# psc0628/NeRF-PRV

Hardware: AMD Instinct MI355X
Metric: ray-samples/s (field evaluations composited; candidate views rendered + scored; scene baseline, field 256^3) (higher is better)
Workload: dtype f16

## Files before the change

### include/prv.h

```cpp
#ifndef PRV_H
#define PRV_H
#include <stddef.h>
#include <stdint.h>

#ifdef __cplusplus
extern "C" {
#endif

#define PRV_ABI_VERSION 5

#define PRV_OK 0
#define PRV_E_INVALID (-1)
#define PRV_E_HIP (-2)
#define PRV_E_IO (-3)
#define PRV_E_NODEVICE (-4)
#define PRV_E_STATE (-5)
#define PRV_E_INTERNAL (-6)

#define PRV_SCORE_ENSEMBLE_RGB 2
#define PRV_SCORE_ENSEMBLE_RGB_DENSITY 3
#define PRV_SCORE_PSNR_COVERAGE 5
#define PRV_SCORE_RAY_ENTROPY 7
#define PRV_SCORE_TERMINATION_JSD 9
#define PRV_TERMINATION_BINS_DEFAULT 16
// ... 241 lines not shown
typedef struct prv_coverage_opts {
  int32_t point_size;
  float depth_tol;
} prv_coverage_opts;
int prv_coverage_default_opts(prv_coverage_opts* opts);
int prv_coverage_create(prv_ctx* ctx, const float* xyz_dev, uint64_t n_points, const prv_camset* cs, const int* view_ids,
                        int n_views, int width, int height, const prv_coverage_opts* opts, float* depth_out_dev,
                        prv_coverage** out);
int prv_coverage_info(const prv_coverage* cov, uint64_t* n_points, int* n_views, uint64_t* n_coverable);
int prv_coverage_visible(const prv_coverage* cov, uint64_t* per_view_host);
int prv_coverage_bits(const prv_coverage* cov, int view, uint64_t* words_host);
int prv_coverage_curve(prv_coverage* cov, const int* order, int k, uint64_t* covered_host, uint32_t* first_seen_dev);
int prv_coverage_greedy(prv_coverage* cov, int k, int* chosen_out, uint64_t* covered_host);
void prv_coverage_destroy(prv_coverage* cov);

int prv_mesh_from_arrays(prv_ctx* ctx, const float* xyz_host, uint64_t n_vertices, const uint32_t* tri_host, uint64_t n_triangles,
                         prv_mesh** out);
int prv_mesh_depth(prv_ctx* ctx, const prv_mesh* m, const prv_camset* cs, const int* view_ids, int n_views, int width, int height,
                   float* depth_out_dev);
int prv_coverage_create_occluded(prv_ctx* ctx, const float* xyz_dev, uint64_t n_points, const prv_mesh* occluder, const prv_camset* cs,
                                 const int* view_ids, int n_views, int width, int height, const prv_coverage_opts* opts,
                                 float* depth_out_dev, prv_coverage** out);

int prv_mesh_set_colors(prv_mesh* m, const uint8_t* rgb_host, uint64_t n_vertices);
int prv_mesh_render(prv_ctx* ctx, const prv_mesh* m, const prv_camset* cs, const int* view_ids, int n_views, int width, int height,
                    int flip180, uint8_t* out_rgba8_dev, float* depth_out_dev, uint32_t* tri_out_dev);

typedef struct prv_comm prv_comm;
int prv_comm_create(prv_ctx* ctx, int rank, int world, const char* transport, const char* rendezvous, prv_comm** out);
void prv_comm_destroy(prv_comm* comm);
int prv_comm_rank(const prv_comm* comm);
int prv_comm_world(const prv_comm* comm);
const char* prv_comm_transport(const prv_comm* comm);
int prv_comm_library(const prv_comm* comm, char* path_out, int path_cap, int* version_out, char* how_out, int how_cap);
int prv_comm_all_gather(prv_comm* comm, const void* send_dev, size_t bytes_per_rank, void* recv_dev);
int prv_comm_barrier(prv_comm* comm);
int prv_shard_views(int n_views, int rank, int world, int interleaved, int* ids_out, int* n_mine);
int prv_score_views_sharded(prv_ctx* ctx, prv_comm* comm, int method, const int* model_slots, int n_models,
                            const prv_camset* cs, int n_views_total, int interleaved, const prv_render_opts* opts,
                            const float* gt_shard_dev, prv_score_record* records_host, prv_stats* stats);
int prv_model_exchange(prv_ctx* ctx, prv_comm* comm, int n_members, const prv_field_desc* desc);
int prv_model_exchange_slots(prv_ctx* ctx, prv_comm* comm, int n_members, const int* slots, const int* owners,
                             const prv_field_desc* desc);

typedef struct prv_train_opts {
  int32_t n_rays;
  int32_t n_samples;
  float lr, beta1, beta2, eps, l2_reg;
  float min_T;
  uint64_t seed;
  int32_t random_bg;
  int32_t occ_every;
  float occ_decay, occ_sigma_thresh;
  int32_t target_samples;
  int32_t patch_w, patch_h;
  int32_t step_mode;
  int32_t deterministic;
} prv_train_opts;
typedef struct prv_trainer prv_trainer;
int prv_train_default_opts(prv_train_opts* opts);
int prv_train_create(prv_ctx* ctx, int model_slot, const prv_camset* dataset, const uint8_t* images_rgba8_dev,
                     int width, int height, const prv_train_opts* opts, prv_trainer** out);
int prv_train_steps(prv_trainer* t, int n_steps, float* losses_host);
int prv_train_steps_multi(prv_trainer** trainers, int n_trainers, int n_steps, float* losses_host);
int prv_train_info(const prv_trainer* t, uint32_t* steps_done, uint64_t* samples_last_batch,
                   uint64_t* table_scalars);
int prv_train_active_rays(const prv_trainer* t);
void prv_train_destroy(prv_trainer* t);
int prv_train_gradients(prv_trainer* t, float* table_grad_host, float* mlp_grad_host, float* loss);
int prv_train_master(prv_trainer* t, float* table_host, float* mlp_host);
int prv_train_refresh_occupancy(prv_trainer* t);
int prv_train_debug_stamps(prv_trainer* t, unsigned long long* out64);

typedef struct prv_model_layout {
  uint64_t table_bytes_canonical;
  uint64_t table_bytes_physical;
  int32_t kernel_features;
  int32_t kernel_dense_levels;
  int32_t n_hashed_levels;
  int32_t kernel_slots;
  int32_t n_dense_levels;
} prv_model_layout;
int prv_debug_model_layout(prv_ctx* ctx, int model_slot, prv_model_layout* out);
int prv_debug_render_clock(prv_ctx* ctx, uint64_t* shader_cycles, uint64_t* ref_ticks, double* ref_hz);
int prv_debug_raygen(prv_ctx* ctx, const prv_camset* cs, int view, int width, int height,
                     int spp_index, float* o, float* d, float* t);
int prv_debug_mesh_stages(prv_ctx* ctx, float ms[4]);
int prv_debug_mesh_component_rounds(const prv_mesh* m, int* rounds);
int prv_debug_raster_stats(prv_ctx* ctx, uint64_t out[2]);
uint64_t prv_debug_live_bytes(void);
int prv_debug_encode(prv_ctx* ctx, int model_slot, const float* pos, int n, uint16_t* feat);
int prv_debug_field(prv_ctx* ctx, int model_slot, const float* pos, const float* dir, int n,
                    float* out36, int32_t* occupied);

#ifdef __cplusplus
}
#endif
#endif
```

### nerf_prv_amd/_lib.py

```python
import ctypes as C
import os

_HERE = os.path.dirname(os.path.abspath(__file__))
LIB_PATH = os.path.join(_HERE, "libprv_hip.so")

PRV_OK = 0
PRV_E_INVALID = -1
PRV_E_HIP = -2
PRV_E_IO = -3
PRV_E_NODEVICE = -4
PRV_E_STATE = -5
PRV_E_INTERNAL = -6

SCORE_ENSEMBLE_RGB = 2
SCORE_ENSEMBLE_RGB_DENSITY = 3
SCORE_PSNR_COVERAGE = 5
SCORE_RAY_ENTROPY = 7
SCORE_TERMINATION_JSD = 9
TERMINATION_BINS_DEFAULT = 16
STEP_FIXED_S = 0
STEP_NGP = 1
NGP_MAX_STEPS = 1024

NN_GRID = 0
# ... 139 lines not shown
    "prv_render_depth": (_i, [_vp, _i, _vp, _vp, _i, _P(RenderOpts), _vp, _vp, _P(Stats)]),
    "prv_render_entropy": (_i, [_vp, _i, _vp, _vp, _i, _P(RenderOpts), _vp, _vp, _P(Stats)]),
    "prv_render_termination": (_i, [_vp, _i, _vp, _vp, _i, _P(RenderOpts), _i, _vp, _vp, _P(Stats)]),
    "prv_termination_divergence": (_i, [_vp, _vp, _vp, _i, _i, _i, _i, _i, _vp, _vp, _vp]),
    "prv_render_footprint": (_i, [_vp, _i, _vp, _vp, _i, _P(RenderOpts), _vp, _vp, _vp, _P(Stats)]),
    "prv_render_surface": (_i, [_vp, _i, _vp, _vp, _i, _P(RenderOpts), C.c_float, _vp, _vp, _vp, _vp, _P(Stats)]),
    "prv_select_default_opts": (_i, [_P(SelectOpts)]),
    "prv_select_from_images": (_i, [_vp, _vp, _vp, _i, _i, _i, _vp, _vp, _vp, _P(SelectOpts), _vp, _vp, _vp, _vp]),
    "prv_select_views": (_i, [_vp, _i, _vp, _vp, _i, _P(RenderOpts), _P(SelectOpts), _vp, _vp, _P(Stats)]),
    "prv_select_views_surface": (_i, [_vp, _i, _vp, _vp, _i, _P(RenderOpts), C.c_float, _P(SelectOpts), _vp, _vp, _P(Stats)]),
    "prv_first_hit": (_i, [_vp, _i, _vp, _vp, _i, _i, _i, C.c_float, _vp]),
    "prv_precept": (_i, [_vp, _i, _vp, _i, _vp, _P(Rs2Intrinsics), C.c_float, _vp]),
    "prv_quantize_rgba8": (_i, [_vp, _vp, C.c_size_t, _vp, _vp]),
    "prv_mesh_default_opts": (_i, [_P(MeshOpts)]),
    "prv_density_grid": (_i, [_vp, _i, _P(MeshOpts), _vp]),
    "prv_marching_cubes": (_i, [_vp, _i, _P(MeshOpts), _P(_vp)]),
    "prv_marching_cubes_grid": (_i, [_vp, _vp, _P(MeshOpts), _P(_vp)]),
    "prv_mesh_counts": (_i, [_vp, _P(C.c_uint64), _P(C.c_uint64)]),
    "prv_mesh_get": (_i, [_vp, _vp, _vp, _vp, _vp]),
    "prv_mesh_save": (_i, [_vp, C.c_char_p, C.c_double, _vp]),
    "prv_mesh_write_file": (_i, [C.c_char_p, C.c_uint64, _vp, _vp, _vp, C.c_uint64, _vp, C.c_double, _vp]),
    "prv_mesh_destroy": (None, [_vp]),
    "prv_mesh_filter_default_opts": (_i, [_P(MeshFilterOpts)]),
    "prv_mesh_components": (_i, [_vp, _P(C.c_uint64)]),
    "prv_mesh_component_info": (_i, [_vp, C.c_uint64, _vp]),
    "prv_mesh_labels": (_i, [_vp, _vp, _vp]),
    "prv_mesh_filter": (_i, [_vp, _P(MeshFilterOpts), _P(_vp)]),
    "prv_mesh_sample": (_i, [_vp, C.c_uint64, C.c_uint64, _vp, _vp]),
    "prv_nn_default_opts": (_i, [_P(NNOpts)]),
    "prv_nn_index_create": (_i, [_vp, _vp, C.c_uint64, _P(NNOpts), _P(_vp)]),
    "prv_nn_query": (_i, [_vp, _vp, C.c_uint64, _vp, _vp]),
    "prv_nn_index_info": (_i, [_vp, _P(C.c_uint64), _P(C.c_int32), _P(C.c_int32)]),
    "prv_debug_nn_tests": (_i, [_vp, _P(C.c_uint64)]),
    "prv_nn_index_destroy": (None, [_vp]),
    "prv_geometry_metrics": (_i, [_vp, _vp, C.c_uint64, _vp, C.c_uint64, C.c_float, _P(GeomMetrics)]),
    "prv_geometry_metrics_indexed": (_i, [_vp, _vp, C.c_uint64, _vp, _vp, C.c_uint64, C.c_float, _P(GeomMetrics)]),
    "prv_coverage_default_opts": (_i, [_P(CoverageOpts)]),
    "prv_coverage_create": (_i, [_vp, _vp, C.c_uint64, _vp, _vp, _i, _i, _i, _P(CoverageOpts), _vp, _P(_vp)]),
    "prv_coverage_info": (_i, [_vp, _P(C.c_uint64), _P(_i), _P(C.c_uint64)]),
    "prv_coverage_visible": (_i, [_vp, _vp]),
    "prv_coverage_bits": (_i, [_vp, _i, _vp]),
    "prv_coverage_curve": (_i, [_vp, _vp, _i, _vp, _vp]),
    "prv_coverage_greedy": (_i, [_vp, _i, _vp, _vp]),
    "prv_coverage_destroy": (None, [_vp]),
    "prv_mesh_from_arrays": (_i, [_vp, _vp, C.c_uint64, _vp, C.c_uint64, _P(_vp)]),
    "prv_mesh_depth": (_i, [_vp, _vp, _vp, _vp, _i, _i, _i, _vp]),
    "prv_mesh_set_colors": (_i, [_vp, _vp, C.c_uint64]),
    "prv_mesh_render": (_i, [_vp, _vp, _vp, _vp, _i, _i, _i, _i, _vp, _vp, _vp]),
    "prv_coverage_create_occluded": (_i, [_vp, _vp, C.c_uint64, _vp, _vp, _vp, _i, _i, _i, _P(CoverageOpts), _vp, _P(_vp)]),
    "prv_debug_raster_stats": (_i, [_vp, _vp]),
    "prv_debug_live_bytes": (C.c_uint64, []),
    "prv_score_ensemble_images": (_i, [_vp, _i, _vp, _i, _i, C.c_size_t, _vp]),
    "prv_score_psnr_images": (_i, [_vp, _vp, _vp, _i, C.c_size_t, _vp, _vp]),
    "prv_evaluate_images": (_i, [_vp, _vp, _vp, _i, _i, _i, _vp, _vp, _vp]),
    "prv_evaluate": (_i, [_vp, _i, _vp, _vp, _i, _P(RenderOpts), _vp, _P(C.c_double), _P(C.c_double)]),
    "prv_score_views": (_i, [_vp, _i, _vp, _i, _vp, _vp, _i, _P(RenderOpts), _vp, _vp, _vp, _P(Stats)]),
    "prv_rank": (_i, [_vp, _vp, _i, _vp]),
    "prv_argmax": (_i, [_vp, _vp, _i]),
    "prv_splat_points": (_i, [_vp, _vp, _vp, C.c_size_t, C.c_double, _vp, _vp, _vp, _i, _i, _i, _i, _i, _vp]),
    "prv_train_default_opts": (_i, [_P(TrainOpts)]),
    "prv_train_create": (_i, [_vp, _i, _vp, _vp, _i, _i, _P(TrainOpts), _P(_vp)]),
    "prv_train_steps": (_i, [_vp, _i, _vp]),
    "prv_train_steps_multi": (_i, [_vp, _i, _i, _vp]),
    "prv_train_debug_stamps": (_i, [_vp, _vp]),
    "prv_train_info": (_i, [_vp, _P(C.c_uint32), _P(C.c_uint64), _P(C.c_uint64)]),
    "prv_train_active_rays": (_i, [_vp]),
    "prv_train_destroy": (None, [_vp]),
    "prv_train_gradients": (_i, [_vp, _vp, _vp, _P(C.c_float)]),
    "prv_train_master": (_i, [_vp, _vp, _vp]),
    "prv_train_refresh_occupancy": (_i, [_vp]),
    "prv_comm_create": (_i, [_vp, _i, _i, C.c_char_p, C.c_char_p, C.POINTER(_vp)]),
    "prv_comm_destroy": (None, [_vp]),
    "prv_comm_rank": (_i, [_vp]),
    "prv_comm_world": (_i, [_vp]),
    "prv_comm_transport": (C.c_char_p, [_vp]),
    "prv_comm_library": (_i, [_vp, C.c_char_p, _i, _P(_i), C.c_char_p, _i]),
    "prv_comm_all_gather": (_i, [_vp, _vp, C.c_size_t, _vp]),
    "prv_comm_barrier": (_i, [_vp]),
    "prv_shard_views": (_i, [_i, _i, _i, _i, _vp, C.POINTER(_i)]),
    "prv_score_views_sharded": (_i, [_vp, _vp, _i, _vp, _i, _vp, _i, _i, C.POINTER(RenderOpts), _vp, _vp, C.POINTER(Stats)]),
    "prv_model_exchange": (_i, [_vp, _vp, _i, C.POINTER(FieldDesc)]),
    "prv_model_exchange_slots": (_i, [_vp, _vp, _i, _P(_i), _P(_i), C.POINTER(FieldDesc)]),
    "prv_debug_model_layout": (_i, [_vp, _i, C.POINTER(ModelLayout)]),
    "prv_debug_render_clock": (_i, [_vp, C.POINTER(C.c_uint64), C.POINTER(C.c_uint64), C.POINTER(C.c_double)]),
    "prv_debug_raygen": (_i, [_vp, _vp, _i, _i, _i, _i, _vp, _vp, _vp]),
    "prv_debug_mesh_stages": (_i, [_vp, _P(C.c_float)]),
    "prv_debug_mesh_component_rounds": (_i, [_vp, _P(C.c_int)]),
    "prv_debug_encode": (_i, [_vp, _i, _vp, _i, _vp]),
    "prv_debug_field": (_i, [_vp, _i, _vp, _vp, _i, _vp, _vp]),
}

_lib = None


def load():
    global _lib
    if _lib is not None:
        return _lib
    if not os.path.exists(LIB_PATH):
        raise ImportError(
            f"{LIB_PATH} is missing: build it with `python -c 'import __graft_entry__ as g; g.build()'` "
            "(hipcc --offload-arch=gfx950). There is no CPU fallback for the render path."
        )
    lib = C.CDLL(LIB_PATH)
    for name, (res, args) in SIGNATURES.items():
        try:
            fn = getattr(lib, name)
        except AttributeError as e:
            raise ImportError(f"{LIB_PATH} does not export {name}") from e
        fn.restype = res
        fn.argtypes = args
    _lib = lib
    return lib


def device_code_digest(path=None):
    import hashlib
    import struct

    path = path or LIB_PATH
    with open(path, "rb") as fh:
        data = fh.read()
    if data[:4] != b"\x7fELF" or data[4] != 2:
        raise ValueError(f"{path} is not a 64-bit ELF file")
    shoff, = struct.unpack_from("<Q", data, 0x28)
    shentsize, shnum, shstrndx = struct.unpack_from("<HHH", data, 0x3A)
    sections = [struct.unpack_from("<IIQQQQIIQQ", data, shoff + i * shentsize) for i in range(shnum)]
    stroff = sections[shstrndx][4]
    for name_off, _type, _flags, _addr, off, size, *_ in sections:
        end = data.index(b"\0", stroff + name_off)
        if data[stroff + name_off:end] == b".hip_fatbin":
            return hashlib.sha256(data[off:off + size]).hexdigest()[:16]
    raise ValueError(f"{path} has no .hip_fatbin section")
```

### nerf_prv_amd/api.py

```python
import ctypes as C
import enum
import json
import math

import numpy as np

from . import _lib as L

RECORD_DTYPE = np.dtype([("score", "<f8"), ("psnr", "<f4"), ("coverage", "<f4")])

FIELD_256 = dict(n_levels=8, n_features=4, log2_hashmap=19, base_res=16, finest_res=256, occ_res=128,
                 density_bias=3.0, table_amp=4.0)
FIELD_512 = dict(n_levels=16, n_features=2, log2_hashmap=21, base_res=16, finest_res=512, occ_res=128,
                 density_bias=3.0, table_amp=4.0)
FIELD_HBM = dict(n_levels=16, n_features=2, log2_hashmap=24, base_res=16, finest_res=2048, occ_res=128,
                 density_bias=3.0, table_amp=4.0)


class RenderMode(enum.IntEnum):

    Shade = 0
    Depth = 1


Shade, Depth = RenderMode.Shade, RenderMode.Depth


class PrvError(RuntimeError):
    def __init__(self, code, msg):
        super().__init__(f"prv error {code}: {msg}")
        self.code = code


def field_desc(**kw):
    d = dict(FIELD_256)
    d.update(kw)
    return L.FieldDesc(**d)


def render_opts(width, height, samples_per_ray=128, spp=1, min_transmittance=1e-4, background=(0.0, 0.0, 0.0, 0.0),
                step_mode=L.STEP_FIXED_S):
    o = L.RenderOpts()
    o.width, o.height, o.samples_per_ray, o.spp = int(width), int(height), int(samples_per_ray), int(spp)
    o.step_mode = int(step_mode)
    o.min_transmittance = float(min_transmittance)
    for k in range(4):
        o.background[k] = float(background[k])
    return o


def engine_render_opts(width, height, samples_per_ray, spp, min_transmittance, background=(0.0, 0.0, 0.0, 0.0)):
    n = int(samples_per_ray)
    return render_opts(width, height, n, spp, min_transmittance, background, step_mode=L.STEP_NGP if n == 0 else L.STEP_FIXED_S)


def select_opts(k=None, grid_res=None, alpha_min=None):
    o = L.SelectOpts()
    if L.load().prv_select_default_opts(C.byref(o)) != 0:
        raise PrvError(L.PRV_E_INVALID, "prv_select_default_opts failed")
    if k is not None:
        o.k = int(k)
    if grid_res is not None:
        o.grid_res = int(grid_res)
    if alpha_min is not None:
        o.alpha_min = float(alpha_min)
    return o


def model_sizes(desc):
    lib = L.load()
    t, m, o = C.c_uint64(), C.c_uint64(), C.c_uint64()
    rc = lib.prv_model_sizes(C.byref(desc), C.byref(t), C.byref(m), C.byref(o))
    if rc != 0:
        raise PrvError(rc, "invalid field descriptor")
    return t.value, m.value, o.value


def _ptr(a):
    if a is None:
        return None
    if isinstance(a, np.ndarray):
        return a.ctypes.data_as(C.c_void_p)
    return C.c_void_p(a.data_ptr())


class _Handle:
    _destroy = None

    def __init__(self, ctx, handle):
        self.ctx, self.handle = ctx, handle

    def _chk(self, rc):
        if rc != 0:
            lib = self.ctx.lib
            msg = (lib.prv_last_error(self.ctx.handle) if self.ctx.handle else None) or b""
            if not (self.handle and msg) or rc == L.PRV_E_STATE:
                msg = lib.prv_last_error(None) or msg
            raise PrvError(rc, msg.decode())

# ... 1101 lines not shown
```

### nerf_prv_amd/csrc/prv_api.cpp

```cpp
#include <hip/hip_runtime.h>

#include <algorithm>
#include <atomic>
#include <chrono>
#include <cmath>
#include <cstdarg>
#include <cstdio>
#include <cstdlib>
#include <cstring>
#include <memory>
#include <new>
#include <stdexcept>
#include <string>
#include <vector>

#include "prv_buffer.hpp"
#include "prv_json.hpp"
#include "prv_kernels.hpp"
#include "prv_mesh.hpp"
#include "prv_geom.hpp"
#include "prv_select.hpp"
#include "prv_coverage.hpp"
#include "prv_raster.hpp"
#include "prv_levels.hpp"
#include "prv_ingp.hpp"
#include "prv_train.hpp"
#include "prv_train_switches.hpp"

using namespace prv;


namespace {

thread_local std::string g_create_error;
std::atomic<int> g_live_contexts{0};
std::atomic<unsigned long long> g_devices_used{0};
std::atomic<bool> g_rccl_loaded{false};

struct Model {
  bool loaded = false;
  bool dirty = false;
  uint64_t generation = 0;
  prv_field_desc desc{};
  FieldDev dev{};
  uint64_t table_halfs = 0, occ_words = 0;
  uint64_t phys_bytes = 0;
  float occ_lo[3] = {0, 0, 0}, occ_hi[3] = {1, 1, 1};
  Buffer table, phys, occ, occ_coarse, frags, frags64, mlp;
};

}

struct prv_camset {
  std::vector<CamDev> cams;
  CamDev* dev = nullptr;
  int device = 0;
  int width = 0, height = 0;
  bool dataset = false;
};

using prv_handle = prv::Handle<struct prv_ctx>;

struct prv_ctx {
  int device = 0;
  int n_cu = 256;
  hipStream_t own_stream = nullptr;
  hipStream_t stream = nullptr;
  std::vector<hipStream_t> idle_queues;
  hipStream_t capture_stream = nullptr;
  BufferPool parked;
  std::string err;
  Model models[PRV_MAX_SLOTS];
  Buffer queue, queue_ext, stage, counters, view_ids, img_f32, partial, records, dbg[6];
  Buffer stage_depth;
  Buffer stage_foot;
  Buffer stage_hit;
  Buffer stage_bins;
  Buffer term_planes;
  Buffer sel_planes, sel_voxel, sel_q, sel_bits, sel_sums;
  Buffer counters_multi, occ_multi;
  int march_multi = -1;
  Buffer img_u8[PRV_MAX_MODELS];
  bool profiling = false;
  std::vector<hipEvent_t> ev_render, ev_march;
  std::vector<hipEvent_t> ev_free;
  std::vector<float> last_render_ms;
  void* pin = nullptr;
  size_t pin_cap = 0;
  hipEvent_t pin_ev = nullptr;
  int blocks_per_cu = -1;
  int cell_cache = -1;
  std::vector<prv_handle*> handles;
  uint64_t raster_stats[2] = {0, 0};
  float mesh_ms[4] = {0, 0, 0, 0};
  int queue_segments = 8;
  int spatial_regions = 1;
  int pool_on = -1;
  int merge_max = -1;
  size_t stage_budget = (size_t)4 << 30;
  size_t queue_budget = (size_t)8 << 30;
  double coverage_weight = PRV_COVERAGE_WEIGHT_DEFAULT;
};

namespace {

int fail(prv_ctx* c, int code, const char* fmt, ...) {
  char buf[512];
  va_list ap;
  va_start(ap, fmt);
  vsnprintf(buf, sizeof(buf), fmt, ap);
  va_end(ap);
  if (c) c->err = buf;
  else g_create_error = buf;
  return code;
}

int caught(prv_ctx* c) noexcept {
  try {
    throw;
  } catch (const std::bad_alloc&) {
    try {
      return fail(c, PRV_E_INTERNAL, "out of host memory");
    } catch (...) {
      return PRV_E_INTERNAL;
    }
  } catch (const std::exception& e) {
    try {
      return fail(c, PRV_E_INTERNAL, "internal error: %s", e.what());
    } catch (...) {
      return PRV_E_INTERNAL;
    }
  } catch (...) {
    return PRV_E_INTERNAL;
  }
}

#define HIPCHK(c, expr)                                                                           \
  do {                                                                                            \
    hipError_t e__ = (expr);                                                                      \
    if (e__ != hipSuccess) return fail((c), PRV_E_HIP, "%s failed: %s", #expr, hipGetErrorString(e__)); \
  } while (0)

int ensure(prv_ctx* c, Buffer& b, size_t bytes) {
  const char* call = "";
  const hipError_t e = prv::ensure(b, bytes, c->stream, c->parked, &call);
  if (e != hipSuccess) return fail(c, PRV_E_HIP, "%s failed: %s", call, hipGetErrorString(e));
  return PRV_OK;
}

int handle_alive(const prv_handle* h, const char* name, const char* the_name) {
  if (!h) return fail(nullptr, PRV_E_INVALID, "%s is NULL", name);
  if (!h->ctx) return fail(nullptr, PRV_E_STATE, "%s's context has been destroyed", the_name);
  return PRV_OK;
}

static_assert(kMaxFieldLevels == kMaxLevels, "level tables of the host and the kernels must agree");

const int kIn[5] = {32, 64, 32, 64, 64};
const int kOut[5] = {64, 16, 64, 64, 16};
const int kOff[5] = {0, 2048, 3072, 5120, 9216};

inline int hidden_k(int s, int h, int j) { return 32 * (s >> 1) + 16 * (s & 1) + 8 * (j >> 2) + 4 * h + (j & 3); }

void prepack_fragments(const uint16_t* mlp, int n_features, std::vector<uint16_t>& frags, bool v64 = false) {
  frags.assign((size_t)kNumFrags * kFragHalfs, 0);
  int f = 0;
  auto emit = [&](int layer, int mt, int s, int (*kmap)(int, int, int)) {
    uint16_t* dst = frags.data() + (size_t)f * kFragHalfs;
    for (int lane = 0; lane < 64; lane++) {
      const int r = lane & 31, h = lane >> 5;
      int out = 32 * mt + r;
      if (v64 && (layer == 1 || layer == 4) && out >= 20 && out < 20 + (layer == 1 ? 1 : 3)) out -= 20;
      for (int j = 0; j < 8; j++) {
        const int k = kmap(s, h, j);
        dst[lane * 8 + j] = out < kOut[layer] ? mlp[kOff[layer] + k * kOut[layer] + out] : (uint16_t)0;
      }
    }
    f++;
  };
  auto k_feat4 = [](int s, int h, int j) { return 4 * (2 * (s * 2 + j / 4) + h) + j % 4; };
  auto k_feat2 = [](int s, int h, int j) { return 2 * (2 * (s * 4 + j / 2) + h) + j % 2; };
  auto k_rgb_in = [](int s, int h, int j) { return s == 0 ? hidden_k(0, h, j) : 16 + 8 * h + j; };
  auto k_canon = [](int s, int h, int j) { return 16 * s + 8 * h + j; };
  for (int mt = 0; mt < 2; mt++)
    for (int s = 0; s < 2; s++)
      emit(0, mt, s, v64 ? (int (*)(int, int, int))k_canon : n_features == 4 ? (int (*)(int, int, int))k_feat4 : (int (*)(int, int, int))k_feat2);
  for (int s = 0; s < 4; s++) emit(1, 0, s, hidden_k);
  for (int mt = 0; mt < 2; mt++)
    for (int s = 0; s < 2; s++) emit(2, mt, s, k_rgb_in);
  for (int mt = 0; mt < 2; mt++)
    for (int s = 0; s < 4; s++) emit(3, mt, s, hidden_k);
  for (int s = 0; s < 4; s++) emit(4, 0, s, hidden_k);
}

uint16_t f2h(float f) {
  _Float16 h = (_Float16)f;
  uint16_t u;
  memcpy(&u, &h, 2);
  return u;
}
uint64_t mix64(uint64_t z) {
  z = (z ^ (z >> 30)) * 0xBF58476D1CE4E5B9ull;
  z = (z ^ (z >> 27)) * 0x94D049BB133111EBull;
  return z ^ (z >> 31);
}
float rng_sym(uint64_t seed, uint64_t stream, uint64_t i, float amp) {
  const uint64_t hsh = mix64(seed + (stream + 1) * 0xD1B54A32D192ED03ull + i * 0x9E3779B97F4A7C15ull);
  const uint32_t u = (uint32_t)(hsh >> 40);
  const float v = (float)u * (1.0f / 8388608.0f) - 1.0f;
  return v * amp;
}
const float kSynthSpheres[4][4] = {
    {0.50f, 0.50f, 0.50f, 0.35f}, {0.80f, 0.50f, 0.62f, 0.13f}, {0.36f, 0.80f, 0.45f, 0.11f}, {0.40f, 0.24f, 0.78f, 0.10f}};

int install_model(prv_ctx* c, int slot, const prv_field_desc& d, const uint16_t* mlp, const uint32_t* occ_host,
                  const uint16_t* table_host ) {
  Model& m = c->models[slot];
  HostLevel lv[kMaxLevels];
  uint64_t total = 0;
  if (compute_levels(d, lv, &total) != 0) return fail(c, PRV_E_INVALID, "invalid field descriptor");
  m.loaded = false;
  m.desc = d;
  m.table_halfs = total * (uint64_t)d.n_features;
  const uint64_t R = (uint64_t)d.occ_res;
  m.occ_words = (R * R * R + 31) / 32;
  int rc;
  if ((rc = ensure(c, m.table, m.table_halfs * 2)) != PRV_OK) return rc;
  if ((rc = ensure(c, m.occ, m.occ_words * 4)) != PRV_OK) return rc;
  if ((rc = ensure(c, m.frags, (size_t)kNumFrags * kFragHalfs * 2)) != PRV_OK) return rc;
  if ((rc = ensure(c, m.frags64, (size_t)kNumFrags * kFragHalfs * 2)) != PRV_OK) return rc;
  if ((rc = ensure(c, m.mlp, PRV_MLP_HALFS * 2)) != PRV_OK) return rc;
  if (table_host) HIPCHK(c, hipMemcpyAsync(m.table.p, table_host, m.table_halfs * 2, hipMemcpyHostToDevice, c->stream));
  HIPCHK(c, hipMemcpyAsync(m.occ.p, occ_host, m.occ_words * 4, hipMemcpyHostToDevice, c->stream));
  {
    const int R = d.occ_res;
    int lo[3] = {R, R, R}, hi[3] = {-1, -1, -1};
    const bool words = R % 32 == 0;
    for (int z = 0; words && z < R; z++)
      for (int y = 0; y < R; y++)
        for (int w = 0; w < R / 32; w++) {
          const uint32_t v = occ_host[((size_t)R * ((size_t)y + (size_t)R * (size_t)z)) / 32 + (size_t)w];
          if (!v) continue;
          lo[0] = std::min(lo[0], 32 * w + __builtin_ctz(v));
          hi[0] = std::max(hi[0], 32 * w + 31 - __builtin_clz(v));
          lo[1] = std::min(lo[1], y);
          hi[1] = std::max(hi[1], y);
          lo[2] = std::min(lo[2], z);
          hi[2] = std::max(hi[2], z);
        }
    for (int z = 0; !words && z < R; z++)
      for (int y = 0; y < R; y++)
        for (int x = 0; x < R; x++) {
          const size_t b = (size_t)x + (size_t)R * ((size_t)y + (size_t)R * (size_t)z);
          if (!((occ_host[b >> 5] >> (b & 31)) & 1u)) continue;
          const int cxyz[3] = {x, y, z};
          for (int a = 0; a < 3; a++) {
            lo[a] = std::min(lo[a], cxyz[a]);
            hi[a] = std::max(hi[a], cxyz[a]);
          }
        }
    for (int a = 0; a < 3; a++) {
      m.occ_lo[a] = hi[a] < 0 ? 2.0f : (float)(lo[a] - 1) / (float)R;
      m.occ_hi[a] = hi[a] < 0 ? -1.0f : (float)(hi[a] + 2) / (float)R;
    }
  }
  std::vector<uint32_t> coarse;
  if (d.occ_res % 4 == 0 && d.occ_res >= 8) {
    const int R = d.occ_res, Rc = R / 4;
    std::vector<uint8_t> blk((size_t)Rc * Rc * Rc, 0);
    const bool words = R % 32 == 0;
    for (int z = 0; words && z < R; z++)
      for (int y = 0; y < R; y++)
        for (int w = 0; w < R / 32; w++) {
          const uint32_t v = occ_host[((size_t)R * ((size_t)y + (size_t)R * (size_t)z)) / 32 + (size_t)w];
          if (!v) continue;
          uint8_t* row = &blk[(size_t)(8 * w) + (size_t)Rc * ((size_t)(y / 4) + (size_t)Rc * (size_t)(z / 4))];
          for (int k = 0; k < 8; k++)
            if ((v >> (4 * k)) & 0xfu) row[k] = 1;
        }
    for (int z = 0; !words && z < R; z++)
      for (int y = 0; y < R; y++)
        for (int x = 0; x < R; x += 32) {
          const size_t bit0 = (size_t)x + (size_t)R * ((size_t)y + (size_t)R * (size_t)z);
          for (int k = 0; k < 32 && x + k < R; k++) {
            const size_t b = bit0 + k;
            if ((occ_host[b >> 5] >> (b & 31)) & 1u) blk[(size_t)((x + k) / 4) + (size_t)Rc * ((size_t)(y / 4) + (size_t)Rc * (size_t)(z / 4))] = 1;
          }
        }
    coarse.assign(((size_t)Rc * Rc * Rc + 31) / 32, 0u);
    for (int z = 0; z < Rc; z++)
      for (int y = 0; y < Rc; y++)
        for (int x = 0; x < Rc; x++) {
          bool any = false;
          for (int dz = -1; dz <= 1 && !any; dz++)
            for (int dy = -1; dy <= 1 && !any; dy++)
              for (int dx = -1; dx <= 1 && !any; dx++) {
// ... 22 lines not shown
  auto ceil_log2 = [](uint32_t v) { uint32_t s = 0; while ((1u << s) < v) s++; return s; };
  for (int l = 0; l < d.n_levels; l++) {
    order[l] = l;
    if (lv[l].hashed) {
      sx[l] = 0;
      psize[l] = lv[l].size;
    } else {
      sx[l] = ceil_log2(lv[l].res + 1);
      psize[l] = 1u << ceil_log2((lv[l].res + 1u) << (2 * sx[l]));
    }
  }
  std::stable_sort(order, order + d.n_levels, [&](int a, int b) { return psize[a] > psize[b]; });
  uint64_t ptotal = 0;
  for (int k = 0; k < d.n_levels; k++) {
    poff[order[k]] = (uint32_t)ptotal;
    ptotal += psize[order[k]];
  }
  if (ptotal * ebytes >= (1ull << 32)) return fail(c, PRV_E_INVALID, "field too large for 32-bit gather offsets");
  if ((rc = ensure(c, m.phys, ptotal * ebytes)) != PRV_OK) return rc;
  m.phys_bytes = ptotal * ebytes;
  HIPCHK(c, hipMemsetAsync(m.phys.p, 0, ptotal * ebytes, c->stream));
  for (int l = 0; l < d.n_levels; l++) {
    RepackLevel R{lv[l].offset, poff[l], lv[l].size, lv[l].res, sx[l], lv[l].hashed};
    HIPCHK(c, launch_repack_level((const uint16_t*)m.table.p, (uint16_t*)m.phys.p, R, d.n_features, c->stream));
  }
  HIPCHK(c, hipStreamSynchronize(c->stream));
  FieldDev& f = m.dev;
  memset(&f, 0, sizeof(f));
  f.table = (const uint16_t*)m.phys.p;
  f.occ = (const uint32_t*)m.occ.p;
  f.occ_coarse = (d.occ_res % 4 == 0 && d.occ_res >= 8) ? (const uint32_t*)m.occ_coarse.p : nullptr;
  f.frags = (const half8*)m.frags.p;
  f.frags64 = (const half8*)m.frags64.p;
  f.n_levels = d.n_levels;
  f.n_features = d.n_features;
  f.occ_res = d.occ_res;
  f.density_bias = d.density_bias;
  for (int a = 0; a < 3; a++) {
    f.occ_lo[a] = m.occ_lo[a];
    f.occ_hi[a] = m.occ_hi[a];
  }
  f.n_dense_levels = 0;
  while (f.n_dense_levels < d.n_levels && !lv[f.n_dense_levels].hashed) f.n_dense_levels++;
  if (getenv("PRV_NO_PAIR")) f.n_dense_levels = 0;
  f.hash_my_b = (2654435761u * ebytes) & 0xffffffu;
  f.hash_mz_b = (805459861u * ebytes) & 0xffffffu;
  f.hash_m_b = (uint32_t)(((1ull << d.log2_hashmap) - 1ull) * ebytes);
  f.hash_shared = 1;
  f.wide_offsets = 0;
  for (int l = 0; l < d.n_levels; l++)
    if (lv[l].hashed && (lv[l].res > lv[l].size || l < f.n_dense_levels)) f.hash_shared = 0;
  if (getenv("PRV_NO_PAIR")) f.hash_shared = 0;
  for (int l = 0; l < d.n_levels; l++) {
    LevelDev& L = f.levels[l];
    L.scale = lv[l].scale;
    L.res_m1 = lv[l].res - 1;
    if (lv[l].res > 4096) return fail(c, PRV_E_INVALID, "level %d has %u vertices per axis (limit 4096)", l, lv[l].res);
    if (lv[l].hashed) {
      if ((uint64_t)(lv[l].size - 1u) * ebytes >= (1ull << 32)) return fail(c, PRV_E_INVALID, "hashed level of 4 GiB or more");
      L.m_b = (lv[l].size - 1u) * ebytes;
      const bool wide = L.m_b >= (1u << 24);
      L.my_b = wide ? 2654435761u * ebytes : (2654435761u * ebytes) & 0xffffffu;
      L.mz_b = wide ? 805459861u * ebytes : (805459861u * ebytes) & 0xffffffu;
      if (wide) {
        f.wide_offsets = 1;
        f.hash_shared = 0;
      }
    } else {
      L.my_b = ebytes << sx[l];
      L.mz_b = ebytes << (2 * sx[l]);
      L.m_b = 0xffffffffu;
      if (L.mz_b >= (1u << 24) || lv[l].res > 4096) return fail(c, PRV_E_INVALID, "dense level too large");
    }
    L.off_b = poff[l] * ebytes;
    L.myz_b = L.my_b + L.mz_b;
    if (lv[l].hashed) {
      if ((L.off_b & 4095u) != 0u || L.res_m1 > 4095u) f.hash_shared = 0;
      L.pack = (L.off_b & ~4095u) | (L.res_m1 & 4095u);
    } else {
      if ((L.off_b & 31u) != 0u || sx[l] > 31u) f.hash_shared = 0;
      L.pack = (L.off_b & ~31u) | (sx[l] & 31u);
    }
  }
  m.loaded = true;
  m.dirty = false;
  return PRV_OK;
}

int republish_model(prv_ctx* c, int slot) {
  Model& m = c->models[slot];
  HIPCHK(c, hipSetDevice(c->device));
  std::vector<uint16_t> mlp(PRV_MLP_HALFS);
  std::vector<uint32_t> occ(m.occ_words);
  HIPCHK(c, hipMemcpyAsync(mlp.data(), m.mlp.p, PRV_MLP_HALFS * 2, hipMemcpyDeviceToHost, c->stream));
  HIPCHK(c, hipMemcpyAsync(occ.data(), m.occ.p, m.occ_words * 4, hipMemcpyDeviceToHost, c->stream));
  HIPCHK(c, hipStreamSynchronize(c->stream));
  const prv_field_desc d = m.desc;
  return install_model(c, slot, d, mlp.data(), occ.data(), nullptr);
}

int model_present(prv_ctx* c, int slot) {
  if (slot < 0 || slot >= PRV_MAX_SLOTS) return fail(c, PRV_E_INVALID, "model slot %d out of range", slot);
  if (!c->models[slot].loaded) return fail(c, PRV_E_STATE, "model slot %d is empty", slot);
  return PRV_OK;
}

int republish_model(prv_ctx* c, int slot);

int check_model(prv_ctx* c, int slot) {
  int rc = model_present(c, slot);
  if (rc != PRV_OK) return rc;
  if (c->models[slot].dirty) return republish_model(c, slot);
  return PRV_OK;
}

int check_opts(prv_ctx* c, const prv_render_opts* o) {
  if (!o) return fail(c, PRV_E_INVALID, "render options are NULL");
  if (o->width < 1 || o->height < 1 || o->width > 16384 || o->height > 16384)
    return fail(c, PRV_E_INVALID, "bad image size %dx%d", o->width, o->height);
  if (o->step_mode != PRV_STEP_FIXED_S && o->step_mode != PRV_STEP_NGP)
    return fail(c, PRV_E_INVALID, "step_mode must be PRV_STEP_FIXED_S (0) or PRV_STEP_NGP (1), got %d", o->step_mode);
  if (o->step_mode == PRV_STEP_FIXED_S && (o->samples_per_ray < 1 || o->samples_per_ray > kMaxSamples))
    return fail(c, PRV_E_INVALID, "samples_per_ray must be in [1,%d], got %d", kMaxSamples, o->samples_per_ray);
  if (o->spp < 1 || o->spp > 1024) return fail(c, PRV_E_INVALID, "spp must be in [1,1024], got %d", o->spp);
  return PRV_OK;
}

int check_surface_level(prv_ctx* c, const prv_render_opts* o, float level) {
  if (!(level > 0.0f && level < 1.0f)) return fail(c, PRV_E_INVALID, "level must be in (0, 1), got %g", (double)level);
  if (1.0f - level < o->min_transmittance)
    return fail(c, PRV_E_INVALID, "level %g: 1 - level = %g is below min_transmittance %g, rays would be cut before they can cross", (double)level,
                (double)(1.0f - level), (double)o->min_transmittance);
  return PRV_OK;
}

int check_device_ptr(prv_ctx* c, const void* p, const char* what) {
  if (!p) return PRV_OK;
  hipPointerAttribute_t a;
  if (hipPointerGetAttributes(&a, p) != hipSuccess) {
    (void)hipGetLastError();
    return fail(c, PRV_E_INVALID, "%s is not a device pointer", what);
  }
  if (a.type != hipMemoryTypeDevice && a.type != hipMemoryTypeManaged && a.type != hipMemoryTypeUnified)
    return fail(c, PRV_E_INVALID, "%s is not a device pointer", what);
  return PRV_OK;
}

hipError_t take_event(prv_ctx* c, hipEvent_t* e) {
  if (!c->ev_free.empty()) {
    *e = c->ev_free.back();
    c->ev_free.pop_back();
    return hipSuccess;
  }
  return hipEventCreate(e);
}

CamDev cam_at(const prv_camset* cs, int i, int w, int h) {
  const CamDev& c = cs->cams[i];
  CamDev r = c;
  const float s = (float)w / (float)cs->width;
  if (cs->dataset) {
    const float sy = (float)h / (float)cs->height;
    r.fx = c.fx * s;
    r.fy = c.fy * sy;
    r.cx = c.cx * s;
    r.cy = c.cy * sy;
// ... 264 lines not shown
    if (!term) planes[n_planes++] = {t.entropy, &c->stage_depth, &RenderPlanesParams::out_entropy};
    planes[n_planes++] = {t.alpha, &c->stage, &RenderPlanesParams::out_alpha};
  }
  const size_t n_bins = term ? (size_t)t.n_bins : 0;
  if (depth) planes[n_planes++] = {t.depth, colour ? &c->stage_depth : &c->stage_foot, &RenderPlanesParams::out_depth};
  if (surface) planes[n_planes++] = {t.hit, &c->stage_hit, &RenderPlanesParams::out_hit};
  const size_t stage_px = (colour ? 16 : 0) + 4 * ((size_t)n_planes + n_bins);
  if (spp > 1) batch = std::min<size_t>(batch, std::max<size_t>(1, c->stage_budget / (npix * stage_px * (size_t)spp)));
  if (batch * npix * (size_t)spp >= (1ull << 32)) batch = ((1ull << 32) - 1) / (npix * (size_t)spp);
  if (batch == 0) return fail(c, PRV_E_INVALID, "image x spp too large");
  const MarchLayout L(c, W, H, spp);
  const size_t seg_cap_max = L.seg_cap(batch);
  if (seg_cap_max * (size_t)L.n_seg >= (1ull << 32)) return fail(c, PRV_E_INVALID, "image x spp too large");
  if ((rc = ensure(c, c->queue, seg_cap_max * (size_t)L.n_seg * kRecordBytes)) != PRV_OK) return rc;
  if (ngp && (rc = ensure(c, c->queue_ext, seg_cap_max * (size_t)L.n_seg * kExtBytes)) != PRV_OK) return rc;
  if (spp > 1 && colour && (rc = ensure(c, c->stage, batch * npix * (size_t)spp * 16)) != PRV_OK) return rc;
  for (int i = 0; i < n_planes && spp > 1; i++)
    if ((rc = ensure(c, *planes[i].stage, batch * npix * (size_t)spp * 4)) != PRV_OK) return rc;
  if (term && spp > 1 && (rc = ensure(c, c->stage_bins, n_bins * batch * npix * (size_t)spp * 4)) != PRV_OK) return rc;

  const int n_blocks = render_blocks(c, m, npix);
  for (size_t b0 = 0; b0 < (size_t)n_views; b0 += batch) {
    const int nb = (int)std::min(batch, (size_t)n_views - b0);
    float* dst_f32 = t.rgba ? t.rgba + b0 * npix * 4 : nullptr;
    uint32_t* dst_u8 = t.rgba8 ? (uint32_t*)t.rgba8 + b0 * npix : nullptr;
    float *dst[4], *target[4];
    for (int i = 0; i < n_planes; i++) {
      dst[i] = planes[i].out + b0 * npix;
      target[i] = spp > 1 ? (float*)planes[i].stage->p : dst[i];
      HIPCHK(c, hipMemsetAsync(target[i], 0, (size_t)nb * npix * (size_t)spp * 4, c->stream));
    }
    const size_t bins_stride = spp > 1 ? (size_t)nb * npix * (size_t)spp : t.bins_stride;
    float* const bins_target = !term ? nullptr : spp > 1 ? (float*)c->stage_bins.p : t.bins + b0 * npix;
    const size_t plane_px = (size_t)nb * npix * (size_t)spp;
    if (n_bins && bins_stride == plane_px) HIPCHK(c, hipMemsetAsync(bins_target, 0, n_bins * plane_px * 4, c->stream));
    else
      for (size_t k = 0; k < n_bins; k++) HIPCHK(c, hipMemsetAsync(bins_target + k * bins_stride, 0, plane_px * 4, c->stream));
    HIPCHK(c, hipMemsetAsync(c->counters.p, 0, b0 == 0 && t.zero_stats ? kCountersBytes : kStatOffset, c->stream));
    MarchParams mp;
    march_common(mp, c, L, o, up, b0, (size_t)nb, stat);
    mp.field = m.dev;
    mp.S = o->samples_per_ray;
    mp.step_mode = o->step_mode;
    mp.queue = c->queue.p;
    mp.queue_ext = (uint4*)c->queue_ext.p;
    mp.queue_count = q_count;
    mp.out_f32 = !colour ? nullptr : spp > 1 ? (float*)c->stage.p : dst_f32;
    mp.out_u8 = spp > 1 ? nullptr : dst_u8;
    if (private_output) {
      const uint64_t tw = 1ull << mp.tile_w_log2, th = 1ull << mp.tile_h_log2;
      uint64_t live_max = 0;
      for (int i = 0; i < nb; i++) {
        const CamDev& cv = up.cams[b0 + i];
        uint64_t w = mp.tiles_x, h = mp.tiles_y;
        if (cv.cull[2] > 0) {
          const uint64_t x0 = (uint64_t)cv.cull[0] / tw, y0 = (uint64_t)cv.cull[1] / th;
          const uint64_t x1 = std::min<uint64_t>(mp.tiles_x, ((uint64_t)cv.cull[2] + tw - 1) / tw);
          const uint64_t y1 = std::min<uint64_t>(mp.tiles_y, ((uint64_t)std::max(cv.cull[3], 0) + th - 1) / th);
          w = x1 > x0 ? x1 - x0 : 0;
          h = y1 > y0 ? y1 - y0 : 0;
        }
        live_max = std::max(live_max, w * h);
      }
      mp.live_grid = 1;
      mp.live_tiles_max = (uint32_t)live_max;
    }
    if ((rc = timed(c, c->ev_march, [&] { HIPCHK(c, launch_march(mp, nb, spp, c->stream)); return PRV_OK; })) != PRV_OK) return rc;
    RenderPlanesParams pp;
    memset(&pp, 0, sizeof(pp));
    pp.r = render_params(c, m, o, L, mp.seg_cap, {mp.queue, mp.queue_ext, mp.queue_count, mp.out_f32, mp.out_u8}, q_head, stat, t.mode);
    for (int i = 0; i < n_planes; i++) pp.*planes[i].slot = target[i];
    pp.cams = mp.cams;
    pp.view_ids = mp.view_ids;
    pp.npix = (uint32_t)npix;
    pp.nb = (uint32_t)nb;
    pp.T_cross = 1.0f - t.level;
    if (term) {
      pp.out_bins = bins_target;
      pp.plane_stride = bins_stride;
      pp.n_bins = (uint32_t)n_bins;
      pp.bin_mul = (uint32_t)(n_bins * 65536u / (size_t)(ngp ? kNgpMaxSteps : o->samples_per_ray));
    }
    if ((rc = timed(c, c->ev_render, [&] {
           HIPCHK(c, n_planes ? launch_render_planes(pp, t.mode, n_blocks, c->stream) : launch_render(pp.r, n_blocks, c->stream));
           return PRV_OK;
         })) != PRV_OK)
      return rc;
    if (spp > 1 && colour) HIPCHK(c, launch_spp_reduce((const float*)c->stage.p, (size_t)nb * npix, spp, o->background, dst_f32, dst_u8, c->stream));
    for (int i = 0; i < n_planes && spp > 1; i++) HIPCHK(c, launch_spp_reduce_depth(target[i], (size_t)nb * npix, spp, dst[i], c->stream));
    for (size_t k = 0; k < n_bins && spp > 1; k++)
      HIPCHK(c, launch_spp_reduce_depth(bins_target + k * bins_stride, (size_t)nb * npix, spp, t.bins + k * t.bins_stride + b0 * npix, c->stream));
  }
  return PRV_OK;
}

int render_ensemble_ngp(prv_ctx* c, const int* slots, int E, const prv_camset* cs, const int* view_ids, int n_views,
                        const prv_render_opts* o, float* scratch_f32, uint8_t* const* out_u8, bool* done) {
  *done = false;
  if (o->step_mode != PRV_STEP_NGP || !march_multi_supported(E) || n_views == 0) return PRV_OK;
  if (c->march_multi == 0) return PRV_OK;
  if (c->march_multi < 0 && E < 3) return PRV_OK;
  const Model& m0 = c->models[slots[0]];
  for (int e = 1; e < E; e++) {
    const Model& m = c->models[slots[e]];
    if (m.desc.occ_res != m0.desc.occ_res || (m.dev.occ_coarse == nullptr) != (m0.dev.occ_coarse == nullptr)) return PRV_OK;
    for (int f = 0; f < e; f++)
      if (slots[f] == slots[e]) return PRV_OK;
  }
  const int W = o->width, H = o->height, spp = o->spp;
  const size_t npix = (size_t)W * H;
  const size_t slot_bytes = kRecordBytes + kExtBytes;
  if ((size_t)n_views * npix * (size_t)spp >= (1ull << 32)) return PRV_OK;
  if ((size_t)n_views * npix * (size_t)spp * slot_bytes > c->queue_budget) return PRV_OK;
  if (spp > 1 && (size_t)n_views * npix * (size_t)spp * 16 > c->stage_budget) return PRV_OK;
  const MarchLayout L(c, W, H, spp);
  const size_t seg_cap = L.seg_cap((size_t)n_views);
  if (seg_cap * (size_t)L.n_seg >= (1ull << 32)) return PRV_OK;
  int rc;
  if ((rc = ensure(c, c->counters, kCountersBytes)) != PRV_OK) return rc;
  if ((rc = ensure(c, c->counters_multi, (size_t)E * kStatOffset)) != PRV_OK) return rc;
  unsigned long long* stat = (unsigned long long*)((char*)c->counters.p + kStatOffset);
  const size_t R = (size_t)m0.desc.occ_res, n_fine = R * R * R, Rc = R / 4, n_coarse = Rc * Rc * Rc;
  if ((rc = ensure(c, c->occ_multi, n_fine + n_coarse + 64)) != PRV_OK) return rc;
  const size_t q_stride = seg_cap * (size_t)L.n_seg * kRecordBytes, x_stride = seg_cap * (size_t)L.n_seg * kExtBytes,
               s_stride = spp > 1 ? (size_t)n_views * npix * (size_t)spp * 16 : 0;
  {
    const size_t grow = (q_stride * (size_t)E > c->queue.bytes ? q_stride * (size_t)E - c->queue.bytes : 0) +
                        (x_stride * (size_t)E > c->queue_ext.bytes ? x_stride * (size_t)E - c->queue_ext.bytes : 0) +
                        (s_stride * (size_t)E > c->stage.bytes ? s_stride * (size_t)E - c->stage.bytes : 0);
    size_t free_b = 0, total_b = 0;
    if (grow && (hipMemGetInfo(&free_b, &total_b) != hipSuccess || grow + ((size_t)2 << 30) > free_b + c->parked.bytes)) return PRV_OK;
  }

  const OccBox box = union_box(c, slots, E);
  Upload up;
  if ((rc = upload_views(c, cs, view_ids, n_views, W, H, box, up)) != PRV_OK) return rc;

  const bool have_coarse = m0.dev.occ_coarse != nullptr;
  {
    OccInterleaveParams ip{};
    ip.n_members = E;
    for (int e = 0; e < E; e++) ip.bits[e] = c->models[slots[e]].dev.occ;
    ip.n_cells = (uint32_t)n_fine;
    ip.out = (uint8_t*)c->occ_multi.p;
    HIPCHK(c, launch_occ_interleave(ip, c->stream));
    if (have_coarse) {
      for (int e = 0; e < E; e++) ip.bits[e] = c->models[slots[e]].dev.occ_coarse;
      ip.n_cells = (uint32_t)n_coarse;
      ip.out = (uint8_t*)c->occ_multi.p + n_fine;
      HIPCHK(c, launch_occ_interleave(ip, c->stream));
    }
  }

  if ((rc = ensure(c, c->queue, q_stride * (size_t)E)) != PRV_OK) return rc;
  if ((rc = ensure(c, c->queue_ext, x_stride * (size_t)E)) != PRV_OK) return rc;
  if (spp > 1 && (rc = ensure(c, c->stage, s_stride * (size_t)E)) != PRV_OK) return rc;
  HIPCHK(c, hipMemsetAsync(c->counters.p, 0, kCountersBytes, c->stream));
  HIPCHK(c, hipMemsetAsync(c->counters_multi.p, 0, (size_t)E * kStatOffset, c->stream));

  MarchMultiParams mp;
  march_common(mp, c, L, o, up, 0, (size_t)n_views, stat);
  mp.occ_bytes = (const uint8_t*)c->occ_multi.p;
  mp.occ_coarse_bytes = have_coarse ? (const uint8_t*)c->occ_multi.p + n_fine : nullptr;
  mp.occ_res = (int)R;
  for (int a = 0; a < 3; a++) {
    mp.occ_lo[a] = box.occ_lo[a];
    mp.occ_hi[a] = box.occ_hi[a];
  }
  mp.n_members = E;
  for (int e = 0; e < E; e++) {
    MarchMember& mm = mp.mem[e];
    mm.queue = (char*)c->queue.p + q_stride * (size_t)e;
    mm.queue_ext = (uint4*)((char*)c->queue_ext.p + x_stride * (size_t)e);
    mm.queue_count = (uint32_t*)((char*)c->counters_multi.p + (size_t)e * kStatOffset) + kMaxSegments * 16;
    mm.out_f32 = spp > 1 ? (float*)((char*)c->stage.p + s_stride * (size_t)e) : scratch_f32;
    mm.out_u8 = spp > 1 ? nullptr : (uint32_t*)out_u8[e];
  }
  if ((rc = timed(c, c->ev_march, [&] { HIPCHK(c, launch_march_multi(mp, n_views, spp, c->stream)); return PRV_OK; })) != PRV_OK) return rc;

  for (int e = 0; e < E; e++) {
    const Model& m = c->models[slots[e]];
    const int n_blocks = render_blocks(c, m, npix);
    uint32_t* q_head = (uint32_t*)((char*)c->counters_multi.p + (size_t)e * kStatOffset);
    const RenderParams rp = render_params(c, m, o, L, mp.seg_cap, mp.mem[e], q_head, stat, kRenderColour);
    if ((rc = timed(c, c->ev_render, [&] { HIPCHK(c, launch_render(rp, n_blocks, c->stream)); return PRV_OK; })) != PRV_OK) return rc;
    if (spp > 1)
      HIPCHK(c, launch_spp_reduce((const float*)mp.mem[e].out_f32, (size_t)n_views * npix, spp, o->background, scratch_f32, (uint32_t*)out_u8[e], c->stream));
  }
  *done = true;
  return PRV_OK;
}

int fetch_stats(prv_ctx* c, const prv_render_opts* o, int n_views, int n_models, prv_stats* st) {
  if (!st) return PRV_OK;
  unsigned long long ev[72] = {0};
  HIPCHK(c, hipMemcpyAsync(ev, (char*)c->counters.p + kStatOffset, sizeof(ev), hipMemcpyDeviceToHost, c->stream));
  HIPCHK(c, hipStreamSynchronize(c->stream));
  st->wave_rounds = ev[1];
  st->rays = (uint64_t)n_views * n_models * o->width * o->height * o->spp;
  st->samples_nominal = st->rays * (uint64_t)(o->step_mode == PRV_STEP_NGP ? kNgpMaxSteps : o->samples_per_ray);
  st->samples_evaluated = ev[0];
  st->samples_live = 0;
  for (int s = 0; s < 8; s++) st->samples_live += ev[8 * (1 + s)];
  return PRV_OK;
}

struct NamedPtr {
  const void* p;
  const char* name;
};
int render_entry(prv_ctx* c, int slot, const prv_camset* cs, const int* view_ids, int n_views, const prv_render_opts* o, prv_stats* st,
                 RenderTargets t, std::initializer_list<NamedPtr> outs, bool missing, const char* bad,
                 float* RenderTargets::*scratch = nullptr, size_t scratch_px = 0) {
  if (!c) return PRV_E_INVALID;
  int rc;
  if ((rc = check_model(c, slot)) != PRV_OK || (rc = check_opts(c, o)) != PRV_OK) return rc;
  if (!cs || n_views < 0 || (missing && n_views > 0)) return fail(c, PRV_E_INVALID, "%s", bad);
  HIPCHK(c, hipSetDevice(c->device));
  for (const NamedPtr& out : outs)
    if ((rc = check_device_ptr(c, out.p, out.name)) != PRV_OK) return rc;
  if (scratch && !(t.*scratch) && n_views > 0) {
    if ((rc = ensure(c, c->img_f32, (size_t)n_views * o->width * o->height * scratch_px)) != PRV_OK) return rc;
    t.*scratch = (float*)c->img_f32.p;
  }
  if ((rc = render_views(c, slot, cs, view_ids, n_views, o, t)) != PRV_OK) return rc;
  return fetch_stats(c, o, n_views, 1, st);
}

int score_blocks(size_t npix) { return (int)std::min<size_t>(64, std::max<size_t>(1, (npix + 4095) / 4096)); }

}


extern "C" {

int prv_abi_version(void) { return PRV_ABI_VERSION; }

int prv_device_count(void) {
  int n = 0;
  if (hipGetDeviceCount(&n) != hipSuccess) return 0;
  return n;
}

const char* prv_last_error(const prv_ctx* ctx) { return ctx ? ctx->err.c_str() : g_create_error.c_str(); }

int prv_create(prv_ctx** out, int device_id) try {
  if (!out) return fail(nullptr, PRV_E_INVALID, "out is NULL");
  *out = nullptr;
  int n = 0;
  hipError_t e = hipGetDeviceCount(&n);
  if (e != hipSuccess || n <= 0)
    return fail(nullptr, PRV_E_NODEVICE, "no HIP device visible (%s): this library has no CPU path",
                e == hipSuccess ? "count = 0" : hipGetErrorString(e));
  if (device_id < 0 || device_id >= n) return fail(nullptr, PRV_E_INVALID, "device %d out of range [0,%d)", device_id, n);
  hipDeviceProp_t prop;
  if ((e = hipSetDevice(device_id)) != hipSuccess || (e = hipGetDeviceProperties(&prop, device_id)) != hipSuccess)
    return fail(nullptr, PRV_E_HIP, "device %d: %s", device_id, hipGetErrorString(e));
  if (!strstr(prop.gcnArchName, "gfx950"))
    return fail(nullptr, PRV_E_NODEVICE, "device %d is %s; this library is built for gfx950 only", device_id, prop.gcnArchName);
  prv_ctx* c = new prv_ctx();
  c->device = device_id;
  c->n_cu = prop.multiProcessorCount > 0 ? prop.multiProcessorCount : 256;
  if ((e = hipStreamCreateWithFlags(&c->own_stream, hipStreamNonBlocking)) != hipSuccess) {
    delete c;
    return fail(nullptr, PRV_E_HIP, "stream create: %s", hipGetErrorString(e));
  }
  c->stream = c->own_stream;
  if (const char* s = getenv("PRV_BLOCKS_PER_CU")) c->blocks_per_cu = std::max(1, atoi(s));
// ... 927 lines not shown
    if (n_views && (rc = score_ensemble_dev(c, method, imgs, n_models, n_views, npix, rec)) != PRV_OK) return rc;
  } else {
    const bool priv = o->spp == 1;
    RenderTargets t;
    t.rgba = (float*)c->img_f32.p;
    t.private_output = priv;
    if ((rc = render_views(c, model_slots[0], cs, view_ids, n_views, o, t)) != PRV_OK) return rc;
    if (n_views && (rc = score_psnr_dev(c, (const float*)c->img_f32.p, gt, n_views, npix, o->background, c->coverage_weight, rec,
                                        priv ? (const CamDev*)c->view_ids.p : nullptr, o->width)) != PRV_OK)
      return rc;
  }
  if (rec_dev && n_views)
    HIPCHK(c, hipMemcpyAsync(rec_dev, rec, (size_t)n_views * sizeof(prv_score_record), hipMemcpyDeviceToDevice, c->stream));
  if (rec_host && n_views) {
    HIPCHK(c, hipMemcpyAsync(rec_host, rec, (size_t)n_views * sizeof(prv_score_record), hipMemcpyDeviceToHost, c->stream));
    HIPCHK(c, hipStreamSynchronize(c->stream));
  }
  return fetch_stats(c, o, n_views, n_models, st);
} catch (...) { return caught(c); }

int prv_argmax(const prv_score_record* r, const int* ids, int n) {
  if (!r || !ids) return -1;
  double best = -1e100;
  int best_id = -1;
  for (int i = 0; i < n; i++)
    if (r[i].score > best) {
      best = r[i].score;
      best_id = ids[i];
    }
  return best_id;
}

int prv_rank(const prv_score_record* r, const int* ids, int n, int* order) try {
  if (n < 0 || (n > 0 && (!r || !ids || !order))) return PRV_E_INVALID;
  std::vector<int> idx(n);
  for (int i = 0; i < n; i++) idx[i] = i;
  std::stable_sort(idx.begin(), idx.end(), [&](int a, int b) {
    const bool na = std::isnan(r[a].score), nb = std::isnan(r[b].score);
    if (na != nb) return nb;
    if (!na && r[a].score != r[b].score) return r[a].score > r[b].score;
    return ids[a] < ids[b];
  });
  for (int i = 0; i < n; i++) order[i] = ids[idx[i]];
  return PRV_OK;
} catch (...) { return caught(nullptr); }


int prv_debug_render_clock(prv_ctx* c, uint64_t* shader_cycles, uint64_t* ref_ticks, double* ref_hz) try {
  if (!c) return PRV_E_INVALID;
  HIPCHK(c, hipSetDevice(c->device));
  if (!shader_cycles || !ref_ticks || !ref_hz) return fail(c, PRV_E_INVALID, "NULL output");
  if (!c->counters.p) return fail(c, PRV_E_STATE, "nothing rendered yet");
  unsigned long long v[2] = {0, 0};
  HIPCHK(c, hipMemcpyAsync(v, (char*)c->counters.p + kStatOffset + 16, 16, hipMemcpyDeviceToHost, c->stream));
  HIPCHK(c, hipStreamSynchronize(c->stream));
  int khz = 0;
  HIPCHK(c, hipDeviceGetAttribute(&khz, hipDeviceAttributeWallClockRate, c->device));
  *shader_cycles = v[0];
  *ref_ticks = v[1];
  *ref_hz = (double)khz * 1e3;
  return PRV_OK;
} catch (...) { return caught(c); }

int prv_debug_model_layout(prv_ctx* c, int slot, prv_model_layout* out) try {
  if (!c) return PRV_E_INVALID;
  int rc = check_model(c, slot);
  if (rc != PRV_OK) return rc;
  if (!out) return fail(c, PRV_E_INVALID, "out is NULL");
  const Model& m = c->models[slot];
  HostLevel lv[kMaxLevels];
  uint64_t total = 0;
  compute_levels(m.desc, lv, &total);
  out->table_bytes_canonical = m.table_halfs * 2;
  out->table_bytes_physical = m.phys_bytes;
  out->kernel_features = m.dev.n_features;
  out->kernel_dense_levels = render_instance_dense_levels(m.dev);
  out->kernel_slots = 64;
  out->n_dense_levels = m.dev.n_dense_levels;
  out->n_hashed_levels = 0;
  for (int l = 0; l < m.desc.n_levels; l++) out->n_hashed_levels += lv[l].hashed ? 1 : 0;
  return PRV_OK;
} catch (...) { return caught(c); }

int prv_debug_raygen(prv_ctx* c, const prv_camset* cs, int view, int W, int H, int spp_k, float* o, float* d, float* t) try {
  if (!c) return PRV_E_INVALID;
  if (!cs || view < 0 || view >= (int)cs->cams.size() || W < 1 || H < 1 || !o || !d || !t)
    return fail(c, PRV_E_INVALID, "bad argument");
  HIPCHK(c, hipSetDevice(c->device));
  const size_t n = (size_t)W * H;
  int rc;
  if ((rc = ensure(c, c->dbg[0], n * 12)) != PRV_OK || (rc = ensure(c, c->dbg[1], n * 12)) != PRV_OK ||
      (rc = ensure(c, c->dbg[2], n * 8)) != PRV_OK)
    return rc;
  HIPCHK(c, launch_debug_raygen(cam_at(cs, view, W, H), W, H, spp_k, (float*)c->dbg[0].p,
                                (float*)c->dbg[1].p, (float*)c->dbg[2].p, c->stream));
  HIPCHK(c, hipMemcpyAsync(o, c->dbg[0].p, n * 12, hipMemcpyDeviceToHost, c->stream));
  HIPCHK(c, hipMemcpyAsync(d, c->dbg[1].p, n * 12, hipMemcpyDeviceToHost, c->stream));
  HIPCHK(c, hipMemcpyAsync(t, c->dbg[2].p, n * 8, hipMemcpyDeviceToHost, c->stream));
  HIPCHK(c, hipStreamSynchronize(c->stream));
  return PRV_OK;
} catch (...) { return caught(c); }

static int debug_field_common(prv_ctx* c, int slot, const float* pos, const float* dir, int n, uint16_t* feat,
                              float* out36, int32_t* occ) {
  int rc;
  if ((rc = check_model(c, slot)) != PRV_OK) return rc;
  if (n < 0 || (n > 0 && !pos)) return fail(c, PRV_E_INVALID, "bad argument");
  if (n == 0) return PRV_OK;
  HIPCHK(c, hipSetDevice(c->device));
  const size_t N = (size_t)n;
  if ((rc = ensure(c, c->dbg[0], N * 12)) != PRV_OK || (rc = ensure(c, c->dbg[1], N * 12)) != PRV_OK ||
      (rc = ensure(c, c->dbg[3], N * 64)) != PRV_OK || (rc = ensure(c, c->dbg[4], N * 144)) != PRV_OK ||
      (rc = ensure(c, c->dbg[5], N * 4)) != PRV_OK)
    return rc;
  HIPCHK(c, hipMemcpyAsync(c->dbg[0].p, pos, N * 12, hipMemcpyHostToDevice, c->stream));
  if (dir) HIPCHK(c, hipMemcpyAsync(c->dbg[1].p, dir, N * 12, hipMemcpyHostToDevice, c->stream));
  HIPCHK(c, launch_debug_field(c->models[slot].dev, (const float*)c->dbg[0].p, dir ? (const float*)c->dbg[1].p : nullptr,
                               n, (uint16_t*)c->dbg[3].p, (float*)c->dbg[4].p, (int32_t*)c->dbg[5].p, c->stream));
  if (feat) HIPCHK(c, hipMemcpyAsync(feat, c->dbg[3].p, N * 64, hipMemcpyDeviceToHost, c->stream));
  if (out36) HIPCHK(c, hipMemcpyAsync(out36, c->dbg[4].p, N * 144, hipMemcpyDeviceToHost, c->stream));
  if (occ) HIPCHK(c, hipMemcpyAsync(occ, c->dbg[5].p, N * 4, hipMemcpyDeviceToHost, c->stream));
  HIPCHK(c, hipStreamSynchronize(c->stream));
  return PRV_OK;
}

int prv_debug_encode(prv_ctx* c, int slot, const float* pos, int n, uint16_t* feat) try {
  if (!c) return PRV_E_INVALID;
  if (!feat && n > 0) return fail(c, PRV_E_INVALID, "feat is NULL");
  return debug_field_common(c, slot, pos, nullptr, n, feat, nullptr, nullptr);
} catch (...) { return caught(c); }

int prv_debug_field(prv_ctx* c, int slot, const float* pos, const float* dir, int n, float* out36, int32_t* occ) try {
  if (!c) return PRV_E_INVALID;
  if (n > 0 && (!dir || !out36)) return fail(c, PRV_E_INVALID, "NULL argument");
  return debug_field_common(c, slot, pos, dir, n, nullptr, out36, occ);
} catch (...) { return caught(c); }

}

#include "prv_train_api.inc"
#include "prv_comm_api.inc"
#include "prv_mesh_api.inc"
#include "prv_geom_api.inc"
#include "prv_select_api.inc"
#include "prv_raster_api.inc"
#include "prv_raster_color_api.inc"
#include "prv_coverage_api.inc"
```

### nerf_prv_amd/csrc/prv_device.hpp

```cpp
#pragma once
#include <utility>
#include <hip/hip_runtime.h>
#include <stdint.h>

namespace prv {

constexpr int kMaxLevels = 16;
constexpr int kNumFrags = 24;
constexpr int kFragHalfs = 64 * 8;
constexpr int kTile = 16;
constexpr int kChunkRays = kTile * kTile;
constexpr float kNgpDt = 1.7320508075688772f / 1024.0f;

typedef _Float16 half8 __attribute__((ext_vector_type(8)));
typedef _Float16 half4 __attribute__((ext_vector_type(4)));
typedef _Float16 half2v __attribute__((ext_vector_type(2)));
typedef float f32x16 __attribute__((ext_vector_type(16)));

struct LevelDev {
  float scale;
  uint32_t res_m1;
  uint32_t my_b, mz_b;
  uint32_t m_b;
  uint32_t off_b;
  uint32_t myz_b;
  uint32_t pack;
};

struct FieldDev {
  const uint16_t* table;
  const uint32_t* occ;
  const uint32_t* occ_coarse;
  const half8* frags;
  const half8* frags64;
  LevelDev levels[kMaxLevels];
  int n_levels, n_features, occ_res;
  int n_dense_levels;
  uint32_t hash_my_b, hash_mz_b, hash_m_b;
  int hash_shared;
  int wide_offsets;
  float density_bias;
  float occ_lo[3], occ_hi[3];
};

struct CamDev {
  float c2w[12];
  float fx, fy, cx, cy;
  float lens[4];
  int cull[4];
};


__device__ __forceinline__ float clamp01(float x) { return fminf(fmaxf(x, 0.0f), 1.0f); }

__device__ __forceinline__ void spp_offset(int k, float& ox, float& oy) {
  float fk = (float)k;
  float a = fmaf(fk, 0.7548776662466927f, 0.5f);
  float b = fmaf(fk, 0.5698402909980532f, 0.5f);
  ox = a - floorf(a);
  oy = b - floorf(b);
}

__device__ __forceinline__ void lens_eval(const float L[4], float x, float y, float& fx, float& fy, float J[4]) {
  const float k1 = L[0], k2 = L[1], p1 = L[2], p2 = L[3];
  const float r2 = fmaf(x, x, y * y);
  const float kr = fmaf(k2, r2, k1);
  const float radial = fmaf(kr, r2, 1.0f);
  const float dk = 2.0f * fmaf(2.0f * k2, r2, k1);
  const float xy = x * y;
  fx = fmaf(x, radial, fmaf(2.0f * p1, xy, p2 * fmaf(2.0f * x, x, r2)));
  fy = fmaf(y, radial, fmaf(p1, fmaf(2.0f * y, y, r2), (2.0f * p2) * xy));
  const float a = 2.0f * fmaf(p1, x, p2 * y);
  J[0] = fmaf(x * x, dk, fmaf(2.0f * p1, y, fmaf(6.0f * p2, x, radial)));
  J[1] = fmaf(xy, dk, a);
  J[2] = J[1];
  J[3] = fmaf(y * y, dk, fmaf(6.0f * p1, y, fmaf(2.0f * p2, x, radial)));
}

constexpr int kLensIters = 8;
__device__ __forceinline__ void lens_undistort(const float L[4], float& px, float& py) {
  const float xd = px, yd = py;
  float x = xd, y = yd;
  for (int it = 0; it < kLensIters; it++) {
    float fx, fy, J[4];
    lens_eval(L, x, y, fx, fy, J);
    const float ex = fx - xd, ey = fy - yd;
    const float det = fmaf(J[0], J[3], -(J[1] * J[2]));
    const float sx = fmaf(J[3], ex, -(J[1] * ey)) / det;
    const float sy = fmaf(J[0], ey, -(J[2] * ex)) / det;
    x -= sx;
    y -= sy;
  }
  px = x;
  py = y;
}

__device__ __forceinline__ bool has_lens(const CamDev& cam) {
  return cam.lens[0] != 0.0f || cam.lens[1] != 0.0f || cam.lens[2] != 0.0f || cam.lens[3] != 0.0f;
}

__device__ __forceinline__ void raygen(const CamDev& cam, int px, int py, float ox, float oy,
                                       float o[3], float d[3]) {
  float dx = (((float)px + ox) - cam.cx) / cam.fx;
  float dy = (((float)py + oy) - cam.cy) / cam.fy;
  if (has_lens(cam)) lens_undistort(cam.lens, dx, dy);
  float v[3];
#pragma unroll
  for (int r = 0; r < 3; r++) {
    const float* m = cam.c2w + r * 4;
    v[r] = fmaf(m[0], dx, fmaf(m[1], dy, m[2]));
    o[r] = m[3];
  }
  float n2 = fmaf(v[0], v[0], fmaf(v[1], v[1], v[2] * v[2]));
  float inv = 1.0f / sqrtf(n2);
#pragma unroll
  for (int r = 0; r < 3; r++) d[r] = v[r] * inv;
}

__device__ __forceinline__ void dataset_to_engine_point(float scale, const float off[3], const float* p, float e[3]) {
  const float q[3] = {fmaf(p[0], scale, off[0]), fmaf(p[1], scale, off[1]), fmaf(p[2], scale, off[2])};
  e[0] = q[1];
  e[1] = q[2];
  e[2] = q[0];
}

// ... 84 lines not shown
  point[0] = depth * x;
  point[1] = depth * y;
  point[2] = depth;
}

__device__ __forceinline__ _Float16 to_half(float x) {
  asm("" : "+v"(x));
  return (_Float16)x;
}

__device__ __forceinline__ void sh4(float x, float y, float z, float o[16]) {
  float xy = x * y, xz = x * z, yz = y * z, x2 = x * x, y2 = y * y, z2 = z * z;
  o[0] = 0.28209479177387814f;
  o[1] = -0.48860251190291987f * y;
  o[2] = 0.48860251190291987f * z;
  o[3] = -0.48860251190291987f * x;
  o[4] = 1.0925484305920792f * xy;
  o[5] = -1.0925484305920792f * yz;
  o[6] = 0.94617469575755997f * z2 - 0.31539156525251999f;
  o[7] = -1.0925484305920792f * xz;
  o[8] = 0.54627421529603959f * x2 - 0.54627421529603959f * y2;
  o[9] = (0.59004358992664352f * y) * (-3.0f * x2 + y2);
  o[10] = (2.8906114426405538f * xy) * z;
  o[11] = (0.45704579946446572f * y) * (1.0f - 5.0f * z2);
  o[12] = (0.3731763325901154f * z) * (5.0f * z2 - 3.0f);
  o[13] = (0.45704579946446572f * x) * (1.0f - 5.0f * z2);
  o[14] = (1.4453057213202769f * z) * (x2 - y2);
  o[15] = (0.59004358992664352f * x) * (-x2 + 3.0f * y2);
}

template <int F> struct EntryWord;
template <> struct EntryWord<4> { typedef uint2 type; };
template <> struct EntryWord<2> { typedef uint32_t type; };
template <int F> struct Entry;
template <> struct Entry<4> {
  uint32_t w[2];
  __device__ __forceinline__ static Entry load(const char* p) {
    const uint2 v = *reinterpret_cast<const uint2*>(p);
    Entry e;
    e.w[0] = v.x;
    e.w[1] = v.y;
    return e;
  }
};
template <> struct Entry<2> {
  uint32_t w[1];
  __device__ __forceinline__ static Entry load(const char* p) {
    Entry e;
    e.w[0] = *reinterpret_cast<const uint32_t*>(p);
    return e;
  }
};

template <int F> struct EntryPair;
template <> struct EntryPair<4> {
  uint32_t w[4];
  __device__ __forceinline__ static EntryPair load(const char* p) {
    const uint4 v = *reinterpret_cast<const uint4*>(p);
    EntryPair e;
    e.w[0] = v.x; e.w[1] = v.y; e.w[2] = v.z; e.w[3] = v.w;
    return e;
  }
};
template <> struct EntryPair<2> {
  uint32_t w[2];
  __device__ __forceinline__ static EntryPair load(const char* p) {
    const uint2 v = *reinterpret_cast<const uint2*>(p);
    EntryPair e;
    e.w[0] = v.x; e.w[1] = v.y;
    return e;
  }
};

__device__ __forceinline__ half2v cvt_pk_f16(float lo, float hi) {
  half2v r;
  asm("v_cvt_pk_f16_f32 %0, %1, %2" : "=v"(r) : "v"(lo), "v"(hi));
  return r;
}

struct HashConsts {
  uint32_t my_b, mz_b, m_b;
  uint32_t wide;
};
enum { kLevelDense = 0, kLevelHashedShared = 1, kLevelGeneric = 2 };

template <int F>
struct CornerCache {
  uint32_t key;
  uint32_t v[8][F / 2];
};

template <int F, int KIND>
__device__ __forceinline__ void encode_level2(const uint16_t* __restrict__ table, const LevelDev& L, const HashConsts& H, float px,
                                              float py, float pz, half2v out[F / 2]) {
  constexpr bool DENSE = KIND == kLevelDense;
  constexpr int ESH = F == 4 ? 3 : 2;
  const float pos[3] = {fmaf(L.scale, px, 0.5f), fmaf(L.scale, py, 0.5f), fmaf(L.scale, pz, 0.5f)};
  uint32_t c0[3];
  half2v wa[3];
#pragma unroll
  for (int a = 0; a < 3; a++) {
    const float w1 = __builtin_amdgcn_fractf(pos[a]);
    wa[a] = cvt_pk_f16(1.0f - w1, w1);
    c0[a] = (uint32_t)(int)pos[a];
  }
  uint32_t vw[8][F / 2];
  uint32_t pk = L.pack;
  if (KIND != kLevelGeneric) asm volatile("" : "+s"(pk));
  if (DENSE) {
    const uint32_t sxl = pk & 31u, off = pk & ~31u;
    const uint32_t my = (uint32_t)(F * 2) << sxl, mz = (uint32_t)(F * 2) << (2u * sxl);
    const char* base0 = reinterpret_cast<const char*>(table) + off;
    const char* base1 = base0 + my;
    const uint32_t b = (c0[0] << ESH) + __umul24(c0[1], my) + __umul24(c0[2], mz);
    const uint32_t bz = b + mz;
#pragma unroll
    for (int q = 0; q < 4; q++) {
      const EntryPair<F> e = EntryPair<F>::load(((q & 1) ? base1 : base0) + ((q >> 1) ? bz : b));
#pragma unroll
      for (int k = 0; k < F / 2; k++) {
        vw[2 * q][k] = e.w[k];
        vw[2 * q + 1][k] = e.w[F / 2 + k];
      }
    }
  } else if (KIND == kLevelHashedShared) {
    const uint32_t res_m1 = pk & 4095u;
    uint32_t c1[3];
#pragma unroll
    for (int a = 0; a < 3; a++) c1[a] = min(c0[a] + 1u, res_m1);
    const char* base = reinterpret_cast<const char*>(table) + (pk & ~4095u);
    const uint32_t tx[2] = {c0[0] << ESH, c1[0] << ESH};
    const uint32_t ty[2] = {__umul24(c0[1], H.my_b) & H.m_b, __umul24(c1[1], H.my_b) & H.m_b};
    const uint32_t tz[2] = {__umul24(c0[2], H.mz_b) & H.m_b, __umul24(c1[2], H.mz_b) & H.m_b};
    {
#pragma unroll
      for (int c = 0; c < 8; c++) {
        const uint32_t byte_off = __builtin_amdgcn_bitop3_b32(tx[c & 1], ty[(c >> 1) & 1], tz[c >> 2], 0x96);
        const Entry<F> e = Entry<F>::load(base + byte_off);
#pragma unroll
        for (int k = 0; k < F / 2; k++) vw[c][k] = e.w[k];
      }
    }
  } else {
    uint32_t c1[3];
#pragma unroll
    for (int a = 0; a < 3; a++) c1[a] = min(c0[a] + 1u, L.res_m1);
    auto mul = [&](uint32_t a, uint32_t b) { return H.wide ? a * b : __umul24(a, b); };
    const uint32_t tx[2] = {(c0[0] << ESH) & L.m_b, (c1[0] << ESH) & L.m_b};
    const uint32_t ty[2] = {mul(c0[1], L.my_b) & L.m_b, mul(c1[1], L.my_b) & L.m_b};
    const uint32_t tz[2] = {(mul(c0[2], L.mz_b) & L.m_b) | L.off_b, (mul(c1[2], L.mz_b) & L.m_b) | L.off_b};
#pragma unroll
    for (int c = 0; c < 8; c++) {
      const uint32_t byte_off = tx[c & 1] ^ ty[(c >> 1) & 1] ^ tz[c >> 2];
      const Entry<F> e = Entry<F>::load(reinterpret_cast<const char*>(table) + byte_off);
#pragma unroll
      for (int k = 0; k < F / 2; k++) vw[c][k] = e.w[k];
    }
  }
  half2v wp[4];
#pragma unroll
  for (int q = 0; q < 4; q++) {
    const half2v wy = {wa[1][q & 1], wa[1][q & 1]}, wz = {wa[2][q >> 1], wa[2][q >> 1]};
    wp[q] = (wa[0] * wy) * wz;
  }
#pragma unroll
  for (int k = 0; k < F / 2; k++) out[k] = half2v{(_Float16)0.0f, (_Float16)0.0f};
#pragma unroll
  for (int c = 0; c < 8; c++) {
    const _Float16 w = wp[c >> 1][c & 1];
    const half2v ww = {w, w};
#pragma unroll
    for (int k = 0; k < F / 2; k++) out[k] = __builtin_elementwise_fma(ww, __builtin_bit_cast(half2v, vw[c][k]), out[k]);
  }
}

template <int F>
struct LevelStage {
  uint32_t vw[8][F / 2];
  half2v wa[3];
};

template <int F>
__device__ __forceinline__ void level_cell(const LevelDev& L, float px, float py, float pz, uint32_t c0[3], half2v wa[3]) {
  const float pos[3] = {fmaf(L.scale, px, 0.5f), fmaf(L.scale, py, 0.5f), fmaf(L.scale, pz, 0.5f)};
#pragma unroll
  for (int a = 0; a < 3; a++) {
    const float w1 = __builtin_amdgcn_fractf(pos[a]);
    wa[a] = cvt_pk_f16(1.0f - w1, w1);
    c0[a] = (uint32_t)(int)pos[a];
  }
}

template <int F>
__device__ __forceinline__ void stage_dense_level(const uint16_t* __restrict__ table, const LevelDev& L, float px, float py, float pz,
// ... 1 lines not shown
  constexpr int ESH = F == 4 ? 3 : 2;
  uint32_t c0[3];
  level_cell<F>(L, px, py, pz, c0, st.wa);
  uint32_t pk = L.pack;
  asm volatile("" : "+s"(pk));
  const uint32_t sxl = pk & 31u, off = pk & ~31u;
  const uint32_t my = (uint32_t)(F * 2) << sxl, mz = (uint32_t)(F * 2) << (2u * sxl);
  const char* base0 = reinterpret_cast<const char*>(table) + off;
  const char* base1 = base0 + my;
  const uint32_t b = (c0[0] << ESH) + __umul24(c0[1], my) + __umul24(c0[2], mz);
  const uint32_t bz = b + mz;
#pragma unroll
  for (int q = 0; q < 4; q++) {
    const EntryPair<F> e = EntryPair<F>::load(((q & 1) ? base1 : base0) + ((q >> 1) ? bz : b));
#pragma unroll
    for (int k = 0; k < F / 2; k++) {
      st.vw[2 * q][k] = e.w[k];
      st.vw[2 * q + 1][k] = e.w[F / 2 + k];
    }
  }
}

template <int F>
__device__ __forceinline__ void stage_hashed_level(const uint16_t* __restrict__ table, const LevelDev& L, const HashConsts& H, float px,
                                                   float py, float pz, CornerCache<F>& cc, half2v wa[3]) {
  constexpr int ESH = F == 4 ? 3 : 2;
  uint32_t c0[3], c1[3];
  level_cell<F>(L, px, py, pz, c0, wa);
  uint32_t pk = L.pack;
  asm volatile("" : "+s"(pk));
  const uint32_t res_m1 = pk & 4095u;
  const uint32_t key = c0[0] | (c0[1] << 10) | (c0[2] << 20);
  if (key != cc.key) {
    cc.key = key;
#pragma unroll
    for (int a = 0; a < 3; a++) c1[a] = min(c0[a] + 1u, res_m1);
    const char* base = reinterpret_cast<const char*>(table) + (pk & ~4095u);
    const uint32_t tx[2] = {c0[0] << ESH, c1[0] << ESH};
    const uint32_t ty[2] = {__umul24(c0[1], H.my_b) & H.m_b, __umul24(c1[1], H.my_b) & H.m_b};
    const uint32_t tz[2] = {__umul24(c0[2], H.mz_b) & H.m_b, __umul24(c1[2], H.mz_b) & H.m_b};
#pragma unroll
    for (int c = 0; c < 8; c++) {
      const uint32_t byte_off = __builtin_amdgcn_bitop3_b32(tx[c & 1], ty[(c >> 1) & 1], tz[c >> 2], 0x96);
      const Entry<F> e = Entry<F>::load(base + byte_off);
#pragma unroll
      for (int k = 0; k < F / 2; k++) cc.v[c][k] = e.w[k];
    }
  }
}

template <int F>
__device__ __forceinline__ void blend_level(const uint32_t vw[8][F / 2], const half2v wa[3], half2v out[F / 2]) {
  half2v wp[4];
#pragma unroll
  for (int q = 0; q < 4; q++) {
    const half2v wy = {wa[1][q & 1], wa[1][q & 1]}, wz = {wa[2][q >> 1], wa[2][q >> 1]};
    wp[q] = (wa[0] * wy) * wz;
  }
#pragma unroll
  for (int k = 0; k < F / 2; k++) out[k] = half2v{(_Float16)0.0f, (_Float16)0.0f};
#pragma unroll
  for (int c = 0; c < 8; c++) {
    const _Float16 w = wp[c >> 1][c & 1];
    const half2v ww = {w, w};
#pragma unroll
    for (int k = 0; k < F / 2; k++) out[k] = __builtin_elementwise_fma(ww, __builtin_bit_cast(half2v, vw[c][k]), out[k]);
  }
}

template <int F, int NDENSE, int... J>
__device__ __forceinline__ void encode_all_levels_cached(const uint16_t* __restrict__ table, const LevelDev* __restrict__ lv,
                                                         const HashConsts& H, float px, float py, float pz, half2v* out,
                                                         CornerCache<F>* cc, std::integer_sequence<int, J...>) {
  constexpr int NH = 32 / F - NDENSE;
  LevelStage<F> ds[NDENSE];
  half2v hwa[NH][3];
  ((J >= NDENSE ? stage_hashed_level<F>(table, lv[J], H, px, py, pz, cc[J >= NDENSE ? J - NDENSE : 0], hwa[J >= NDENSE ? J - NDENSE : 0]) : (void)0), ...);
  ((J < NDENSE ? stage_dense_level<F>(table, lv[J], px, py, pz, ds[J < NDENSE ? J : 0]) : (void)0), ...);
  __builtin_amdgcn_sched_barrier(0);
  ((J < NDENSE ? blend_level<F>(ds[J < NDENSE ? J : 0].vw, ds[J < NDENSE ? J : 0].wa, out + J * (F / 2))
               : blend_level<F>(cc[J >= NDENSE ? J - NDENSE : 0].v, hwa[J >= NDENSE ? J - NDENSE : 0], out + J * (F / 2))), ...);
}

template <int F, int NDENSE, int... J>
__device__ __forceinline__ void encode_all_levels(const uint16_t* __restrict__ table, const LevelDev* __restrict__ lv, const HashConsts& H,
                                                  float px, float py, float pz, half2v* out, std::integer_sequence<int, J...>) {
  (encode_level2<F, (J < NDENSE ? kLevelDense : NDENSE > 0 ? kLevelHashedShared : kLevelGeneric)>(table, lv[J], H, px, py, pz, out + J * (F / 2)), ...);
}

template <int F, int NDENSE, bool CACHE = false>
__device__ __forceinline__ void encode_sample(const uint16_t* __restrict__ table, const LevelDev* __restrict__ lv, const HashConsts& H,
                                              float px, float py, float pz, half8 f[4], CornerCache<F>* cc = nullptr) {
  px = clamp01(px);
  py = clamp01(py);
  pz = clamp01(pz);
  half2v out[16];
  if constexpr (CACHE && NDENSE > 0) encode_all_levels_cached<F, NDENSE>(table, lv, H, px, py, pz, out, cc, std::make_integer_sequence<int, 32 / F>{});
  else encode_all_levels<F, NDENSE>(table, lv, H, px, py, pz, out, std::make_integer_sequence<int, 32 / F>{});
#pragma unroll
  for (int s = 0; s < 4; s++)
#pragma unroll
    for (int k = 0; k < 4; k++) {
      f[s][2 * k] = out[4 * s + k][0];
      f[s][2 * k + 1] = out[4 * s + k][1];
    }
}

__device__ __forceinline__ void swap_halves(half8& a, half8& b) {
  typedef uint32_t u32x4 __attribute__((ext_vector_type(4)));
  u32x4 x = __builtin_bit_cast(u32x4, a), y = __builtin_bit_cast(u32x4, b);
#pragma unroll
  for (int k = 0; k < 4; k++) {
    const auto r = __builtin_amdgcn_permlane32_swap(x[k], y[k], false, false);
    x[k] = r[0];
    y[k] = r[1];
  }
  a = __builtin_bit_cast(half8, x);
  b = __builtin_bit_cast(half8, y);
}

__device__ __forceinline__ void stage_levels(const FieldDev& fd, LevelDev* lds_levels) {
  static_assert(sizeof(LevelDev) == 32, "LevelDev must be two 16-byte words");
  if (threadIdx.x < (unsigned)fd.n_levels) lds_levels[threadIdx.x] = fd.levels[threadIdx.x];
}


__device__ __forceinline__ f32x16 mfma(half8 a, half8 b, f32x16 c) {
  return __builtin_amdgcn_mfma_f32_32x32x16_f16(a, b, c, 0, 0, 0);
}

template <bool RELU>
__device__ __forceinline__ half8 pack8(const f32x16& acc, int base) {
  half8 r;
#pragma unroll
  for (int j = 0; j < 8; j += 2) {
    half2v p;
    p[0] = (_Float16)acc[base + j];
    p[1] = (_Float16)acc[base + j + 1];
    if (RELU) {
      const half2v z = {(_Float16)0.0f, (_Float16)0.0f};
      p = __builtin_elementwise_max(p, z);
    }
    r[j] = p[0];
    r[j + 1] = p[1];
  }
  return r;
}

struct MlpOut {
  f32x16 dens;
  f32x16 rgb;
};

struct MlpNoTap {
  __device__ __forceinline__ void operator()(int, const half8*) const {}
};

template <class Tap = MlpNoTap>
__device__ __forceinline__ MlpOut mlp_forward(const half8* __restrict__ wl, int lane, half8 f0,
                                              half8 f1, half8 shfrag, Tap tap = Tap()) {
  const f32x16 zero = {0, 0, 0, 0, 0, 0, 0, 0, 0, 0, 0, 0, 0, 0, 0, 0};
  MlpOut out;
  half8 hf[4];
  {
    f32x16 a0 = mfma(wl[0 * 64 + lane], f0, zero);
    f32x16 a1 = mfma(wl[2 * 64 + lane], f0, zero);
    a0 = mfma(wl[1 * 64 + lane], f1, a0);
    a1 = mfma(wl[3 * 64 + lane], f1, a1);
    hf[0] = pack8<true>(a0, 0);
    hf[1] = pack8<true>(a0, 8);
    hf[2] = pack8<true>(a1, 0);
    hf[3] = pack8<true>(a1, 8);
    tap(0, hf);
  }
  {
    f32x16 a = mfma(wl[4 * 64 + lane], hf[0], zero);
    a = mfma(wl[5 * 64 + lane], hf[1], a);
    a = mfma(wl[6 * 64 + lane], hf[2], a);
    a = mfma(wl[7 * 64 + lane], hf[3], a);
    out.dens = a;
  }
// ... 150 lines not shown
```

### nerf_prv_amd/csrc/prv_kernels.hip

```cpp
#include "prv_kernels.hpp"

#include <algorithm>

#ifndef PRV_ABLATE
#define PRV_ABLATE 0
#endif

namespace prv {


__device__ __forceinline__ void morton16(uint32_t i, uint32_t& x, uint32_t& y) {
  x = (i & 1u) | ((i >> 1) & 2u) | ((i >> 2) & 4u) | ((i >> 3) & 8u);
  y = ((i >> 1) & 1u) | ((i >> 2) & 2u) | ((i >> 3) & 4u) | ((i >> 4) & 8u);
}

__device__ __forceinline__ uint32_t march_ngp(const FieldDev& fd, const float o[3], const float d[3], float t0, float t1,
                                              uint32_t (*mw)[256], int& k_lo, int& k_hi, int& first_nz, int& last_nz) {
  const float dt = kNgpDt;
  first_nz = 32;
  last_nz = -1;
  k_lo = k_hi = 0;
  float ta = t0, tb = t1;
#pragma unroll
  for (int a = 0; a < 3; a++) {
// ... 480 lines not shown
#pragma unroll
    for (int e = 0; e < E; e++) {
      k2_lo = min(k2_lo, first_nz[e]);
      k2_hi = max(k2_hi, last_nz[e]);
    }
    uint32_t acc[E][4];
#pragma unroll
    for (int e = 0; e < E; e++)
#pragma unroll
      for (int q = 0; q < 4; q++) acc[e][q] = 0u;
    for (int k = k2_lo; k <= k2_hi; k++) {
      uint32_t w[E];
      bool behind = false;
#pragma unroll
      for (int e = 0; e < E; e++) behind = behind || (k - first_nz[e] >= kWin && k <= last_nz[e]);
      if (!((passmask >> k) & 1u)) {
#pragma unroll
        for (int e = 0; e < E; e++) w[e] = 0u;
      } else if (behind) {
        fine_word(k, w);
      } else {
#pragma unroll
        for (int e = 0; e < E; e++) {
          const int j = k - first_nz[e];
          w[e] = (j >= 0 && k <= last_nz[e]) ? mw[e][j][threadIdx.x] : 0u;
        }
      }
#pragma unroll
      for (int e = 0; e < E; e++) {
        const int j = k - first_nz[e];
        if (j < 0 || k > last_nz[e]) continue;
        const int q = j & 3;
        if (j < 4) {
#pragma unroll
          for (int u = 0; u < 4; u++)
            if (q == u) m[e][u] = w[e];
        } else {
#pragma unroll
          for (int u = 0; u < 4; u++)
            if (q == u) acc[e][u] = w[e];
          if ((q == 3 || k == last_nz[e]) && !(PRV_ABLATE & 128)) {
            const uint32_t slot = base[e] + (uint32_t)__popcll(b[e] & ((1ull << lane) - 1ull));
            P.mem[e].queue_ext[(size_t)((j >> 2) - 1) * ext_stride + slot] = make_uint4(acc[e][0], acc[e][1], acc[e][2], acc[e][3]);
#pragma unroll
            for (int u = 0; u < 4; u++) acc[e][u] = 0u;
          }
        }
      }
    }
  }
#pragma unroll
  for (int e = 0; e < E; e++) {
    const MarchSink Q{P.mem[e].queue, P.mem[e].queue_ext, ext_stride, P.mem[e].queue_count, P.mem[e].out_f32, P.mem[e].out_u8};
    march_write<true, true>(P, Q, stage, r, first_nz[e] < 32, b[e], base[e], dt, m[e], first_nz[e], last_nz[e], [](int) { return 0u; });
  }
}

__global__ __launch_bounds__(256) void occ_interleave_kernel(OccInterleaveParams P) {
  const uint32_t c = blockIdx.x * 256u + threadIdx.x;
  if (c >= P.n_cells) return;
  uint32_t v = 0u;
  for (int e = 0; e < P.n_members; e++) v |= ((P.bits[e][c >> 5] >> (c & 31u)) & 1u) << e;
  P.out[c] = (uint8_t)v;
}


__device__ __forceinline__ void clock_stamp_begin(unsigned long long* stat) {
  if (blockIdx.x == 0 && threadIdx.x == 0) {
    stat[4] = __builtin_readcyclecounter();
    stat[5] = __builtin_amdgcn_s_memrealtime();
  }
}
__device__ __forceinline__ void clock_stamp_end(unsigned long long* stat) {
  if (blockIdx.x == 0 && threadIdx.x == 0) {
    atomicAdd(stat + 2, __builtin_readcyclecounter() - stat[4]);
    atomicAdd(stat + 3, __builtin_amdgcn_s_memrealtime() - stat[5]);
  }
}

__device__ __forceinline__ int lane_id() { return (int)(threadIdx.x & 63u); }

__device__ __forceinline__ float entropy_add(float p, float H) { return p >= 1.17549435e-38f ? fmaf(p, -__builtin_amdgcn_logf(p), H) : H; }

template <int F, int NDENSE, bool NGP, bool CACHE, int MODE>
__device__ __forceinline__ void render_queue64_body(RenderParams P, const RenderPlanesParams* X) {
  using M = RenderMode<MODE>;
  constexpr int kDWord = M::kDWord, kMoveWords = M::kMoveWords, kFrags = M::kFrags;
  __shared__ half8 wl[kFrags * 64];
  __shared__ uint32_t mv[4][32][kMoveWords];
  constexpr uint32_t kPoolCap = 192;
  __shared__ uint32_t pool[kPoolCap][kMoveWords];
  __shared__ uint32_t pool_n, pool_lock;
  for (int i = threadIdx.x; i < kFrags * 64; i += 256) wl[i] = P.field.frags64[i];
  if (threadIdx.x == 0) {
    pool_n = 0u;
    pool_lock = 0u;
  }
  __syncthreads();
  auto pool_acquire = [&]() {
    if (lane_id() == 0)
      while (atomicCAS(&pool_lock, 0u, 1u) != 0u) __builtin_amdgcn_s_sleep(2);
    __builtin_amdgcn_fence(__ATOMIC_ACQUIRE, "workgroup");
    __builtin_amdgcn_wave_barrier();
  };
  auto pool_release = [&]() {
    __builtin_amdgcn_fence(__ATOMIC_RELEASE, "workgroup");
    __builtin_amdgcn_wave_barrier();
    if (lane_id() == 0) atomicExch(&pool_lock, 0u);
  };
  const LevelDev* __restrict__ lvl = P.field.levels;
  const HashConsts hc = {P.field.hash_my_b, P.field.hash_mz_b, P.field.hash_m_b, (uint32_t)P.field.wide_offsets};

  const int lane = threadIdx.x & 63, r = lane & 31, g = lane >> 5;

  bool active = false;
  uint32_t pix = 0, rec_i = 0;
  float o[3] = {0, 0, 0}, d[3] = {0, 0, 1}, t0 = 0.f, dt = 0.f;
  uint32_t cur = 0, m1 = 0, m2 = 0, m3 = 0, base = 0;
  float T = 1.f, cr = 0.f, cg = 0.f, cb = 0.f;
  float D = 0.f;
  float Hs = 0.f;
  uint32_t tbin = 0u;
  half8 shA = {0, 0, 0, 0, 0, 0, 0, 0}, shB = {0, 0, 0, 0, 0, 0, 0, 0};
  bool drained = false;
  unsigned long long n_eval = 0ull, n_rounds = 0ull;
  constexpr int kCached = CACHE ? 32 / F - NDENSE : 1;
  CornerCache<F> cc[kCached];
#pragma unroll
  for (int j = 0; j < kCached; j++) cc[j].key = ~0u;
  clock_stamp_begin(P.stat_evaluated);
  uint32_t q_cur = 0, q_end = 0;
  const uint32_t n_seg = (uint32_t)P.n_segments;
  const uint32_t n_sub = (uint32_t)max(P.n_sub, 1);
  uint32_t seg = n_seg > 1u ? (((uint32_t)__builtin_amdgcn_s_getreg((3 << 11) | 20) & 7u) % (n_seg / n_sub)) * n_sub + (blockIdx.x * 4u + (threadIdx.x >> 6)) % n_sub : 0u;
  uint32_t seg_tried = 0;
  const uint4* __restrict__ queue = reinterpret_cast<const uint4*>(P.queue);

  auto take_ray = [&](uint32_t ri, uint32_t next) {
    const uint4* rec = queue + (size_t)ri * kRecordWords;
    const uint4 q0 = rec[0], q1 = rec[1], q3 = rec[3];
    uint4 mk = rec[2];
    o[0] = __uint_as_float(q0.x); o[1] = __uint_as_float(q0.y); o[2] = __uint_as_float(q0.z);
    t0 = __uint_as_float(q0.w);
    d[0] = __uint_as_float(q1.x); d[1] = __uint_as_float(q1.y); d[2] = __uint_as_float(q1.z);
    dt = __uint_as_float(q1.w);
    pix = q3.x;
    rec_i = ri;
    base = 0u;
    if constexpr (NGP) {
      const uint32_t base0 = q3.y & 0xffffu;
      base = base0;
      if (next >= base0 + 128u) {
        const uint32_t j = (next - base0) >> 7;
        mk = P.queue_ext[(size_t)(j - 1u) * ((size_t)P.seg_cap * (size_t)P.n_segments) + (size_t)ri];
        base = base0 + 128u * j;
      }
    }
    cur = mk.x; m1 = mk.y; m2 = mk.z; m3 = mk.w;
    while (base + 32u <= next) {
      cur = m1; m1 = m2; m2 = m3; m3 = 0u;
      base += 32u;
    }
    if (next > base) cur &= ~0u << (next & 31u);
    while (cur == 0u && (m1 | m2 | m3) != 0u) {
      cur = m1; m1 = m2; m2 = m3; m3 = 0u;
      base += 32u;
    }
    active = true;
// ... 130 lines not shown
          }
          if (g == grp) {
            T = __uint_as_float(ent[2]);
            if constexpr (M::ENTROPY) {
              Hs = __uint_as_float(ent[3]);
            } else {
              cr = __uint_as_float(ent[3]); cg = __uint_as_float(ent[4]); cb = __uint_as_float(ent[5]);
            }
            if constexpr (M::DSTATE) D = __uint_as_float(ent[kDWord]);
            if constexpr (M::TERM) tbin = ent[4];
            take_ray(ent[0], ent[1]);
          }
        }
      }
    }
    const unsigned long long idle = __ballot(!active);
    const bool needA = (uint32_t)idle == 0xffffffffu, needB = (uint32_t)(idle >> 32) == 0xffffffffu;
    if (!drained && (needA || needB)) {
#pragma unroll
      for (int grp = 0; grp < 2; grp++) {
        if (!(grp == 0 ? needA : needB)) continue;
        while (q_cur == q_end && !drained) {
          uint32_t claim = 0;
          if (lane == 0) claim = atomicAdd(P.queue_head + 16u * seg, kClaim);
          claim = __builtin_amdgcn_readfirstlane(claim);
          const uint32_t s_lo = seg * P.seg_cap, s_cnt = min(P.queue_count[16u * seg], P.seg_cap) - P.queue_count[16u * seg + 1u];
          if (claim < s_cnt) {
            q_cur = s_lo + claim;
            q_end = min(q_cur + kClaim, s_lo + s_cnt);
          } else if (++seg_tried >= n_seg) {
            drained = true;
          } else {
            seg = seg + 1u == n_seg ? 0u : seg + 1u;
          }
        }
        const uint32_t avail = min(32u, q_end - q_cur);
        if ((uint32_t)r < avail) {
          if constexpr (!M::ENTROPY) {
            const half8 sh = reinterpret_cast<const half8*>(queue + (size_t)(q_cur + (uint32_t)r) * kRecordWords)[4 + g];
            if (grp == 0) shA = sh;
            else shB = sh;
          }
          if (g == grp) {
            T = 1.f; cr = 0.f; cg = 0.f; cb = 0.f;
            if constexpr (M::DSTATE) D = 0.f;
            if constexpr (M::ENTROPY) Hs = 0.f;
            if constexpr (M::TERM) tbin = 0u;
            take_ray(q_cur + (uint32_t)r, 0u);
          }
        }
        q_cur += avail;
      }
    }
    const unsigned long long act = __ballot(active);
    if (act == 0ull) {
      if (drained && (!P.pool_on || *(volatile uint32_t*)&pool_n == 0u)) break;
      continue;
    }
    n_eval += (unsigned long long)__popcll(act);
    n_rounds += 2ull;

    half8 f[4];
#pragma unroll
    for (int s = 0; s < 4; s++) asm volatile("" : "=v"(f[s]));
    bool last = false;
    float ts = 0.f;
    uint32_t sbin = 0u;
    if (active) {
      const uint32_t i = base + (uint32_t)__builtin_ctz(cur);
      cur &= cur - 1u;
      if (cur == 0u) {
        last = (m1 | m2 | m3) == 0u;
        while (cur == 0u && !last) {
          cur = m1; m1 = m2; m2 = m3; m3 = 0u;
          base += 32u;
        }
        if constexpr (NGP) {
          if (last) last = !next_chunk();
        }
      }
      const float t = fmaf((float)i + 0.5f, dt, t0);
      if constexpr (M::DSTATE) ts = t;
      if constexpr (M::TERM) sbin = min((i * X->bin_mul) >> 16, X->n_bins - 1u);
      encode_sample<F, NDENSE, CACHE>(P.field.table, lvl, hc, fmaf(t, d[0], o[0]), fmaf(t, d[1], o[1]), fmaf(t, d[2], o[2]), f, cc);
    }
    swap_halves(f[0], f[1]);
    swap_halves(f[2], f[3]);
    const half8 fA[2] = {f[0], f[2]}, fB[2] = {f[1], f[3]};
    MlpOut2 mo;
    if constexpr (M::ENTROPY) mlp_density2(wl, lane, fA, fB, mo.densA, mo.densB);
    else mo = mlp_forward2(wl, lane, fA, fB, shA, shB);
    const float dens = g ? mo.densB[8] : mo.densA[0];
    float lr = 0.f, lg = 0.f, lb = 0.f;
    if constexpr (!M::ENTROPY) {
      lr = g ? mo.rgbB[8] : mo.rgbA[0];
      lg = g ? mo.rgbB[9] : mo.rgbA[1];
      lb = g ? mo.rgbB[10] : mo.rgbA[2];
    }

    bool done = false;
    if (active) {
      const float sigma = fast_exp(dens + P.field.density_bias);
      const float alpha = 1.0f - fast_exp(-(sigma * dt));
      const float wgt = alpha * T;
      if constexpr (M::TERM) {
        if (sbin != tbin) {
          X->out_bins[(size_t)tbin * X->plane_stride + pix] = Hs;
          Hs = 0.f;
          tbin = sbin;
        }
        Hs = Hs + wgt;
      } else if constexpr (M::ENTROPY) {
        Hs = entropy_add(wgt, Hs);
      } else {
        cr = fmaf(wgt, fast_sigmoid(lr), cr);
        cg = fmaf(wgt, fast_sigmoid(lg), cg);
        cb = fmaf(wgt, fast_sigmoid(lb), cb);
      }
      if constexpr (M::DEPTH) D = fmaf(wgt, ts, D);
      T = T * (1.0f - alpha);
      if constexpr (M::SURF) {
        if (D == 0.f && T <= X->T_cross) D = ts;
      }
      done = last || T < P.min_T;
    }
    if (done) {
      if constexpr (!M::ENTROPY) {
        const float4 v = make_float4(cr, cg, cb, 1.0f - T);
        reinterpret_cast<float4*>(P.out_f32)[pix] = v;
        if (P.last_pass && P.out_u8) P.out_u8[pix] = quantize_rgba8(v.x, v.y, v.z, v.w, P.bg);
      }
      if constexpr (M::TERM) {
        X->out_bins[(size_t)tbin * X->plane_stride + pix] = Hs;
        X->out_alpha[pix] = 1.0f - T;
      } else if constexpr (M::ENTROPY) {
        X->out_entropy[pix] = entropy_add(T, Hs);
        X->out_alpha[pix] = 1.0f - T;
      }
      if constexpr (M::DSTATE) {
        const CamDev& cam = X->cams[X->view_ids[(pix / X->npix) % X->nb]];
        const float fx = cam.c2w[2], fy = cam.c2w[6], fz = cam.c2w[10];
        const float inv = 1.0f / sqrtf(fmaf(fx, fx, fmaf(fy, fy, fz * fz)));
        X->out_depth[pix] = D * (fmaf(d[0], fx, fmaf(d[1], fy, d[2] * fz)) * inv);
        if constexpr (M::SURF) X->out_hit[pix] = D > 0.f ? 1.0f : 0.0f;
      }
      active = false;
    }
  }
  if (lane == 0 && n_eval) {
    atomicAdd(P.stat_evaluated, n_eval);
    atomicAdd(P.stat_evaluated + 1, n_rounds);
  }
  clock_stamp_end(P.stat_evaluated);
}

template <int F, int NDENSE, bool NGP, bool CACHE = false>
__global__ __launch_bounds__(256)
__attribute__((amdgpu_waves_per_eu(CACHE ? 2 : NDENSE == 0 ? 1 : 3)))
void render_queue64_kernel(RenderParams P) {
  render_queue64_body<F, NDENSE, NGP, CACHE, kRenderColour>(P, nullptr);
}

template <int F, int NDENSE, bool NGP, int MODE>
__global__ __launch_bounds__(256)
__attribute__((amdgpu_waves_per_eu(NDENSE == 0 ? 1 : MODE == kRenderSurface && F == 4 && !NGP ? 4 : 3)))
void render_planes_kernel(RenderPlanesParams P) {
  render_queue64_body<F, NDENSE, NGP, false, MODE>(P.r, &P);
}

__device__ __forceinline__ int32_t first_hit_dda(const FieldDev& fd, const float o[3], const float d[3], float max_range) {
  float t0, t1;
  int32_t result = -1;
  if (ray_aabb(o, d, t0, t1)) {
    if (t1 > max_range) t1 = max_range;
    if (t1 > t0) {
      const int R = fd.occ_res;
      const float fR = (float)R;
      const float ts = t0 + 1e-6f;
      int c[3], step[3];
      float tmax[3], tdelta[3];
#pragma unroll
      for (int a = 0; a < 3; a++) {
        const float p = clamp01(fmaf(ts, d[a], o[a])) * fR;
        c[a] = min((int)p, R - 1);
        if (d[a] > 0.f) {
          step[a] = 1;
          tmax[a] = (((float)(c[a] + 1)) / fR - o[a]) / d[a];
          tdelta[a] = 1.0f / (fR * d[a]);
        } else if (d[a] < 0.f) {
          step[a] = -1;
          tmax[a] = (((float)c[a]) / fR - o[a]) / d[a];
          tdelta[a] = -1.0f / (fR * d[a]);
        } else {
          step[a] = 0;
          tmax[a] = __builtin_inff();
          tdelta[a] = __builtin_inff();
        }
      }
      for (;;) {
        const uint32_t bit = (uint32_t)c[0] + (uint32_t)R * ((uint32_t)c[1] + (uint32_t)R * (uint32_t)c[2]);
        if ((fd.occ[bit >> 5] >> (bit & 31)) & 1u) {
          result = (int32_t)bit;
          break;
        }
        const int a = tmax[0] < tmax[1] ? (tmax[0] < tmax[2] ? 0 : 2) : (tmax[1] < tmax[2] ? 1 : 2);
        const float tm = a == 0 ? tmax[0] : (a == 1 ? tmax[1] : tmax[2]);
        if (tm > t1) break;
        if (a == 0) { c[0] += step[0]; tmax[0] += tdelta[0]; if (c[0] < 0 || c[0] >= R) break; }
        else if (a == 1) { c[1] += step[1]; tmax[1] += tdelta[1]; if (c[1] < 0 || c[1] >= R) break; }
        else { c[2] += step[2]; tmax[2] += tdelta[2]; if (c[2] < 0 || c[2] >= R) break; }
      }
    }
  }
  return result;
}

__global__ __launch_bounds__(256) void first_hit_kernel(FieldDev fd, const CamDev* __restrict__ cams, int W, int H,
                                                        float max_range, int32_t* __restrict__ out) {
  const int i = blockIdx.x * 256 + threadIdx.x;
  if (i >= W * H) return;
  const int v = blockIdx.y;
  const int px = i % W, py = i / W;
  float o[3], d[3], t0, t1;
  raygen(cams[v], px, py, 0.5f, 0.5f, o, d);
  (void)t0;
  (void)t1;
  const int32_t result = first_hit_dda(fd, o, d, max_range);
  out[(size_t)v * W * H + i] = result;
}

__global__ __launch_bounds__(256) void precept_kernel(FieldDev fd, const float* __restrict__ voxels, int n, PreceptPose pose,
                                                      Rs2Intr in, float max_range, int32_t* __restrict__ out) {
  const int i = blockIdx.x * 256 + threadIdx.x;
  if (i >= n) return;
  const float origin[3] = {(float)pose.c2w[3], (float)pose.c2w[7], (float)pose.c2w[11]};
  double v[3];
#pragma unroll
  for (int r = 0; r < 3; r++)
    v[r] = pose.w2c[r * 4] * (double)voxels[i * 3] + pose.w2c[r * 4 + 1] * (double)voxels[i * 3 + 1] +
           pose.w2c[r * 4 + 2] * (double)voxels[i * 3 + 2] + pose.w2c[r * 4 + 3];
  const float point_3d[3] = {(float)v[0], (float)v[1], (float)v[2]};
  float pixel[2];
  rs2_project(pixel, in, point_3d);
// ... 330 lines not shown
                                     double* __restrict__ out) {
  const int v = blockIdx.x * blockDim.x + threadIdx.x;
  if (v >= n_views) return;
  double s = 0.0;
  for (int b = 0; b < n_blocks; b++) s += partial[(size_t)v * n_blocks + b];
  out[v] = s / count;
}

__global__ void score_finalize_kernel(const double* __restrict__ partial, int n_views, int n_blocks,
                                      int method, size_t pixels_per_view, double coverage_weight,
                                      prv_score_record* __restrict__ rec) {
  const int v = blockIdx.x * blockDim.x + threadIdx.x;
  if (v >= n_views) return;
  prv_score_record out;
  out.psnr = 0.f;
  out.coverage = 0.f;
  if (method == PRV_SCORE_PSNR_COVERAGE) {
    double se = 0.0, cov = 0.0, unc = 0.0;
    for (int b = 0; b < n_blocks; b++) {
      se += partial[((size_t)v * n_blocks + b) * 3 + 0];
      cov += partial[((size_t)v * n_blocks + b) * 3 + 1];
      unc += partial[((size_t)v * n_blocks + b) * 3 + 2];
    }
    const double mse = se / (double)(pixels_per_view * 3);
    const double psnr = -10.0 * log10(mse);
    out.score = -psnr + coverage_weight * (unc / (double)pixels_per_view);
    out.psnr = (float)psnr;
    out.coverage = (float)(cov / (double)pixels_per_view);
  } else if (method == PRV_SCORE_RAY_ENTROPY) {
    double sh = 0.0, sa = 0.0;
    for (int b = 0; b < n_blocks; b++) {
      sh += partial[((size_t)v * n_blocks + b) * 2 + 0];
      sa += partial[((size_t)v * n_blocks + b) * 2 + 1];
    }
    out.score = sh / (double)pixels_per_view;
    out.coverage = (float)(sa / (double)pixels_per_view);
  } else {
    double s = 0.0;
    for (int b = 0; b < n_blocks; b++) s += partial[(size_t)v * n_blocks + b];
    out.score = s;
  }
  rec[v] = out;
}


__device__ __forceinline__ unsigned long long mix64(unsigned long long z) {
  z = (z ^ (z >> 30)) * 0xBF58476D1CE4E5B9ull;
  z = (z ^ (z >> 27)) * 0x94D049BB133111EBull;
  return z ^ (z >> 31);
}

__global__ __launch_bounds__(256) void synth_table_kernel(uint16_t* __restrict__ table, size_t n,
                                                          unsigned long long seed, float amp) {
  for (size_t i = (size_t)blockIdx.x * 256 + threadIdx.x; i < n; i += (size_t)gridDim.x * 256) {
    unsigned long long hsh = mix64(seed + 1ull * 0xD1B54A32D192ED03ull + (unsigned long long)i * 0x9E3779B97F4A7C15ull);
    uint32_t u = (uint32_t)(hsh >> 40);
    float v = (float)u * (1.0f / 8388608.0f) - 1.0f;
    _Float16 hv = to_half(v * amp);
    table[i] = __builtin_bit_cast(uint16_t, hv);
  }
}

template <int F>
__global__ __launch_bounds__(256) void repack_level_kernel(const uint16_t* __restrict__ canon,
                                                           uint16_t* __restrict__ phys, RepackLevel L) {
  typedef typename EntryWord<F>::type word_t;
  const word_t* src = reinterpret_cast<const word_t*>(canon) + L.canon_off;
  word_t* dst = reinterpret_cast<word_t*>(phys) + L.phys_off;
  if (L.hashed) {
    for (uint32_t i = blockIdx.x * 256 + threadIdx.x; i < L.n; i += gridDim.x * 256) dst[i] = src[i];
    return;
  }
  const uint32_t nv = L.res * L.res * L.res;
  for (uint32_t i = blockIdx.x * 256 + threadIdx.x; i < nv; i += gridDim.x * 256) {
    const uint32_t x = i % L.res, y = (i / L.res) % L.res, z = i / (L.res * L.res);
    const word_t v = src[i];
    const uint32_t ex = x == L.res - 1 ? 1u : 0u, ey = y == L.res - 1 ? 1u : 0u, ez = z == L.res - 1 ? 1u : 0u;
    for (uint32_t dz = 0; dz <= ez; dz++)
      for (uint32_t dy = 0; dy <= ey; dy++)
        for (uint32_t dx = 0; dx <= ex; dx++) dst[(x + dx) | ((y + dy) << L.sx) | ((z + dz) << (2 * L.sx))] = v;
  }
}


__global__ __launch_bounds__(256) void debug_raygen_kernel(CamDev cam, int W, int H, int spp_k,
                                                           float* __restrict__ o_out,
                                                           float* __restrict__ d_out,
                                                           float* __restrict__ t_out) {
  const int i = blockIdx.x * 256 + threadIdx.x;
  if (i >= W * H) return;
  const int px = i % W, py = i / W;
  float ox, oy, o[3], d[3], t0, t1;
  spp_offset(spp_k, ox, oy);
  raygen(cam, px, py, ox, oy, o, d);
  ray_aabb(o, d, t0, t1);
  for (int a = 0; a < 3; a++) {
    o_out[i * 3 + a] = o[a];
    d_out[i * 3 + a] = d[a];
  }
  t_out[i * 2] = t0;
  t_out[i * 2 + 1] = t1;
}

template <int F, int NDENSE>
__global__ __launch_bounds__(256) void debug_field64_kernel(FieldDev fd, const float* __restrict__ pos, const float* __restrict__ dir,
                                                            int n, uint16_t* __restrict__ feat, float* __restrict__ out36,
                                                            int32_t* __restrict__ occ_out) {
  __shared__ half8 wl[kNumFrags * 64];
  const LevelDev* __restrict__ lvl = fd.levels;
  for (int i = threadIdx.x; i < kNumFrags * 64; i += 256) wl[i] = fd.frags64[i];
  __syncthreads();
  const int lane = threadIdx.x & 63, r = lane & 31, g = lane >> 5;
  const int wave = blockIdx.x * 4 + (threadIdx.x >> 6);
  const int idx = wave * 64 + lane, idxA = wave * 64 + r, idxB = idxA + 32;
  const bool ok = idx < n;
  float p[3] = {0.5f, 0.5f, 0.5f};
  if (ok)
    for (int a = 0; a < 3; a++) p[a] = pos[idx * 3 + a];
  auto dir_of = [&](int i, float dd[3]) {
    dd[0] = 0.f; dd[1] = 0.f; dd[2] = 1.f;
    if (dir && i < n)
      for (int a = 0; a < 3; a++) dd[a] = dir[i * 3 + a];
  };
  float dA[3], dB[3];
  dir_of(idxA, dA);
  dir_of(idxB, dB);
  half8 f[4];
  const HashConsts hc = {fd.hash_my_b, fd.hash_mz_b, fd.hash_m_b, (uint32_t)fd.wide_offsets};
  encode_sample<F, NDENSE>(fd.table, lvl, hc, p[0], p[1], p[2], f);
  if (ok && feat) {
    typedef uint16_t ushort8 __attribute__((ext_vector_type(8)));
    uint16_t* dst = feat + (size_t)idx * 32;
#pragma unroll
    for (int s = 0; s < 4; s++) {
      const ushort8 u = __builtin_bit_cast(ushort8, f[s]);
#pragma unroll
      for (int e = 0; e < 8; e++) dst[8 * s + e] = u[e];
    }
  }
  swap_halves(f[0], f[1]);
  swap_halves(f[2], f[3]);
  const half8 fA[2] = {f[0], f[2]}, fB[2] = {f[1], f[3]};
  const MlpOut2 mo = mlp_forward2(wl, lane, fA, fB, sh_fragment(g, dA[0], dA[1], dA[2]), sh_fragment(g, dB[0], dB[1], dB[2]));
  if (out36) {
    if (ok) {
      float* q = out36 + (size_t)idx * 36;
      q[0] = fast_exp((g ? mo.densB[8] : mo.densA[0]) + fd.density_bias);
      q[1] = fast_sigmoid(g ? mo.rgbB[8] : mo.rgbA[0]);
      q[2] = fast_sigmoid(g ? mo.rgbB[9] : mo.rgbA[1]);
      q[3] = fast_sigmoid(g ? mo.rgbB[10] : mo.rgbA[2]);
    }
#pragma unroll
    for (int i = 0; i < 8; i++) {
      const int row = (i & 3) + 8 * (i >> 2) + 4 * g;
      if (idxA < n) {
        out36[(size_t)idxA * 36 + 4 + row] = mo.densA[i];
        out36[(size_t)idxA * 36 + 20 + row] = mo.rgbA[i];
      }
      if (idxB < n) {
        out36[(size_t)idxB * 36 + 4 + row] = mo.densB[i];
        out36[(size_t)idxB * 36 + 20 + row] = mo.rgbB[i];
      }
    }
  }
  if (ok && occ_out) occ_out[idx] = occupied(fd, p[0], p[1], p[2]) ? 1 : 0;
}



__global__ __launch_bounds__(256) void splat_points_kernel(const float* __restrict__ xyz, const uint8_t* __restrict__ rgb,
                                                           size_t n, float scale, float ox, float oy, float oz,
                                                           const CamDev* __restrict__ cams, int W, int H, int point_size,
                                                           unsigned long long* __restrict__ zbuf) {
  const size_t i = (size_t)blockIdx.x * 256 + threadIdx.x;
  if (i >= n) return;
  const CamDev cam = cams[blockIdx.y];
  const float off[3] = {ox, oy, oz};
  const float p[3] = {xyz[3 * i], xyz[3 * i + 1], xyz[3 * i + 2]};
  float e[3], u, v, z;
  dataset_to_engine_point(scale, off, p, e);
  if (!project_engine_point(cam, e, u, v, z)) return;
  const uint32_t col = (uint32_t)rgb[3 * i] | ((uint32_t)rgb[3 * i + 1] << 8) | ((uint32_t)rgb[3 * i + 2] << 16);
  const unsigned long long key = ((unsigned long long)__float_as_uint(z) << 32) | col;
  const int x0 = (int)floorf(u - 0.5f * (float)point_size + 0.5f), y0 = (int)floorf(v - 0.5f * (float)point_size + 0.5f);
  unsigned long long* zb = zbuf + (size_t)blockIdx.y * W * H;
  for (int dy = 0; dy < point_size; dy++)
    for (int dx = 0; dx < point_size; dx++) {
      const int x = x0 + dx, y = y0 + dy;
      if (x < 0 || y < 0 || x >= W || y >= H) continue;
      atomicMin(zb + (size_t)y * W + x, key);
    }
}

__global__ __launch_bounds__(256) void splat_resolve_kernel(const unsigned long long* __restrict__ zbuf, int W, int H,
                                                            int flip180, uint32_t* __restrict__ out) {
  const size_t npix = (size_t)W * H;
  const size_t i = (size_t)blockIdx.x * 256 + threadIdx.x;
  if (i >= npix) return;
  const unsigned long long k = zbuf[(size_t)blockIdx.y * npix + i];
  uint32_t px = 0x00ffffffu;
  if (k != ~0ull) {
    const uint32_t col = (uint32_t)k & 0x00ffffffu;
    px = col | (col == 0x00ffffffu ? 0u : 0xff000000u);
  }
  const int x = (int)(i % W), y = (int)(i / W);
  const size_t o = flip180 ? ((size_t)(H - 1 - y) * W + (size_t)(W - 1 - x)) : i;
  out[(size_t)blockIdx.y * npix + o] = px;
}


hipError_t launch_splat_points(const float* xyz, const uint8_t* rgb, size_t n, float scale, const float off[3],
                               const CamDev* cams, int n_views, int W, int H, int point_size, int flip180,
                               unsigned long long* zbuf, uint32_t* out, hipStream_t s) {
  hipError_t e = hipMemsetAsync(zbuf, 0xff, (size_t)n_views * W * H * 8, s);
  if (e != hipSuccess) return e;
  if (n > 0)
    hipLaunchKernelGGL(splat_points_kernel, dim3((unsigned)((n + 255) / 256), n_views), dim3(256), 0, s, xyz, rgb, n, scale,
                       off[0], off[1], off[2], cams, W, H, point_size, zbuf);
  hipLaunchKernelGGL(splat_resolve_kernel, dim3((unsigned)(((size_t)W * H + 255) / 256), n_views), dim3(256), 0, s, zbuf, W, H,
                     flip180, out);
  return hipGetLastError();
}

hipError_t launch_spp_reduce(const float* stage, size_t n_pixels, int spp, const float bg[4], float* out, uint32_t* out_u8,
                             hipStream_t s) {
  unsigned blocks = (unsigned)std::min<size_t>(4096, (n_pixels + 255) / 256);
  hipLaunchKernelGGL(spp_reduce_kernel, dim3(blocks), dim3(256), 0, s, reinterpret_cast<const float4*>(stage), n_pixels, spp,
                     1.0f / (float)spp, bg[0], bg[1], bg[2], bg[3], reinterpret_cast<float4*>(out), out_u8);
  return hipGetLastError();
}

hipError_t launch_spp_reduce_depth(const float* stage, size_t n_pixels, int spp, float* out, hipStream_t s) {
  unsigned blocks = (unsigned)std::min<size_t>(4096, (n_pixels + 255) / 256);
  if (blocks == 0) return hipSuccess;
  hipLaunchKernelGGL(spp_reduce_depth_kernel, dim3(blocks), dim3(256), 0, s, stage, n_pixels, spp, 1.0f / (float)spp, out);
  return hipGetLastError();
}

hipError_t launch_march(const MarchParams& P, int n_views, int n_spp, hipStream_t s) {
  dim3 grid((unsigned)(P.live_grid ? P.live_tiles_max : P.tiles_x * P.tiles_y), (unsigned)n_views, (unsigned)(P.spp_inner_log2 > 0 ? 1 : n_spp));
  if (grid.x == 0) return hipSuccess;
  if (!P.out_f32) {
    if (P.step_mode == PRV_STEP_NGP) hipLaunchKernelGGL(march_compact_noimage_kernel<true>, grid, dim3(256), 0, s, P);
    else hipLaunchKernelGGL(march_compact_noimage_kernel<false>, grid, dim3(256), 0, s, P);
    return hipGetLastError();
  }
  if (P.step_mode == PRV_STEP_NGP) hipLaunchKernelGGL(march_compact_kernel<true>, grid, dim3(256), 0, s, P);
  else hipLaunchKernelGGL(march_compact_kernel<false>, grid, dim3(256), 0, s, P);
  return hipGetLastError();
}

hipError_t launch_occ_interleave(const OccInterleaveParams& P, hipStream_t s) {
  hipLaunchKernelGGL(occ_interleave_kernel, dim3((P.n_cells + 255u) / 256u), dim3(256), 0, s, P);
  return hipGetLastError();
}

bool march_multi_supported(int n_members) { return n_members == 2 || n_members == 5; }

hipError_t launch_march_multi(const MarchMultiParams& P, int n_views, int n_spp, hipStream_t s) {
  dim3 grid((unsigned)(P.tiles_x * P.tiles_y), (unsigned)n_views, (unsigned)(P.spp_inner_log2 > 0 ? 1 : n_spp));
  if (grid.x == 0) return hipSuccess;
  if (P.n_members == 5) hipLaunchKernelGGL((march_multi_kernel<5, 8>), grid, dim3(256), 0, s, P);
  else if (P.n_members == 2) hipLaunchKernelGGL((march_multi_kernel<2, 12>), grid, dim3(256), 0, s, P);
  else return hipErrorInvalidValue;
  return hipGetLastError();
}

template <bool NGP>
static void launch_render_mode(const RenderParams& P, int n_blocks, hipStream_t s) {
  if (P.cell_cache && P.field.n_features == 4 && render_instance_dense_levels(P.field) == 5) {
    hipLaunchKernelGGL((render_queue64_kernel<4, 5, NGP, true>), dim3(n_blocks), dim3(256), 0, s, P);
    return;
  }
  with_field_instance(P.field, [&](auto f, auto nd) {
    hipLaunchKernelGGL((render_queue64_kernel<decltype(f)::value, decltype(nd)::value, NGP>), dim3(n_blocks), dim3(256), 0, s, P);
  });
}

hipError_t launch_render(const RenderParams& P, int n_blocks, hipStream_t s) {
  if (P.step_mode == PRV_STEP_NGP) launch_render_mode<true>(P, n_blocks, s);
  else launch_render_mode<false>(P, n_blocks, s);
  return hipGetLastError();
}

template <int MODE>
static void launch_render_planes_mode(const RenderPlanesParams& P, int n_blocks, hipStream_t s) {
  with_field_instance(P.r.field, [&](auto f, auto nd) {
    constexpr int F = decltype(f)::value, ND = decltype(nd)::value;
    if (P.r.step_mode == PRV_STEP_NGP) hipLaunchKernelGGL((render_planes_kernel<F, ND, true, MODE>), dim3(n_blocks), dim3(256), 0, s, P);
    else hipLaunchKernelGGL((render_planes_kernel<F, ND, false, MODE>), dim3(n_blocks), dim3(256), 0, s, P);
  });
}

hipError_t launch_render_planes(const RenderPlanesParams& P, int mode, int n_blocks, hipStream_t s) {
  if (mode == kRenderDepth) launch_render_planes_mode<kRenderDepth>(P, n_blocks, s);
  else if (mode == kRenderEntropy) launch_render_planes_mode<kRenderEntropy>(P, n_blocks, s);
  else if (mode == kRenderFootprint) launch_render_planes_mode<kRenderFootprint>(P, n_blocks, s);
  else if (mode == kRenderSurface) launch_render_planes_mode<kRenderSurface>(P, n_blocks, s);
  else if (mode == kRenderTermination) launch_render_planes_mode<kRenderTermination>(P, n_blocks, s);
  else return hipErrorInvalidValue;
  return hipGetLastError();
}

hipError_t launch_score_entropy(const float* entropy, const float* alpha, size_t npix, int n_views, int n_blocks, double* partial,
                                hipStream_t s) {
  hipLaunchKernelGGL(score_entropy_kernel, dim3((unsigned)n_blocks, (unsigned)n_views), dim3(256), 0, s, entropy, alpha, npix, partial);
  return hipGetLastError();
}

hipError_t launch_score_termination_jsd(const TerminationJsdParams& P, int n_views, int n_blocks, hipStream_t s) {
  hipLaunchKernelGGL(score_termination_jsd_kernel, dim3((unsigned)n_blocks, (unsigned)n_views), dim3(256), 0, s, P);
  return hipGetLastError();
}

hipError_t launch_first_hit(const FieldDev& fd, const CamDev* cams, int n_views, int W, int H, float max_range,
                            int32_t* out, hipStream_t s) {
  dim3 grid((unsigned)((W * H + 255) / 256), (unsigned)n_views);
  hipLaunchKernelGGL(first_hit_kernel, grid, dim3(256), 0, s, fd, cams, W, H, max_range, out);
  return hipGetLastError();
}

hipError_t launch_precept(const FieldDev& fd, const float* voxels, int n, const PreceptPose& pose, const Rs2Intr& in,
                          float max_range, int32_t* out, hipStream_t s) {
  hipLaunchKernelGGL(precept_kernel, dim3((unsigned)((n + 255) / 256)), dim3(256), 0, s, fd, voxels, n, pose, in, max_range, out);
  return hipGetLastError();
}

hipError_t launch_quantize(const float* in, size_t n, const float bg[4], uint8_t* out, hipStream_t s) {
  unsigned blocks = (unsigned)((n + 255) / 256);
  if (blocks > 4096) blocks = 4096;
  if (blocks == 0) blocks = 1;
  hipLaunchKernelGGL(quantize_kernel, dim3(blocks), dim3(256), 0, s, reinterpret_cast<const float4*>(in), n,
                     bg[0], bg[1], bg[2], bg[3], reinterpret_cast<uint32_t*>(out));
  return hipGetLastError();
}

hipError_t launch_score_ensemble(const EnsembleParams& P, int method, int n_views, int n_blocks, prv_score_record* rec,
                                 hipStream_t s) {
  dim3 grid((unsigned)n_blocks, (unsigned)n_views);
  const size_t n_terms = P.pixels_per_view * (method == PRV_SCORE_ENSEMBLE_RGB ? 3 : 2);
  if (method == PRV_SCORE_ENSEMBLE_RGB)
    hipLaunchKernelGGL(score_ensemble_terms_kernel<PRV_SCORE_ENSEMBLE_RGB>, grid, dim3(256), 0, s, P);
  else
    hipLaunchKernelGGL(score_ensemble_terms_kernel<PRV_SCORE_ENSEMBLE_RGB_DENSITY>, grid, dim3(256), 0, s, P);
  hipLaunchKernelGGL(score_sequential_sum_kernel, dim3((unsigned)n_views), dim3(64), 0, s, (const double*)P.partial, n_terms,
                     rec + P.view0);
  return hipGetLastError();
}

hipError_t launch_score_psnr(const PsnrParams& P, int n_views, int n_blocks, hipStream_t s) {
  dim3 grid((unsigned)n_blocks, (unsigned)n_views);
  hipLaunchKernelGGL(score_psnr_kernel, grid, dim3(256), 0, s, P);
  return hipGetLastError();
}

hipError_t launch_ssim(const float* img, const float* gt, int n_views, int W, int H, const float bg[4], float* la,
                       float* lb, double* partial, int n_blocks, double* out, hipStream_t s) {
  const size_t n = (size_t)n_views * W * H;
  unsigned blocks = (unsigned)std::min<size_t>(4096, (n + 255) / 256);
  hipLaunchKernelGGL(ssim_lum_kernel, dim3(blocks), dim3(256), 0, s, reinterpret_cast<const float4*>(img),
                     reinterpret_cast<const float4*>(gt), n, bg[0], bg[1], bg[2], bg[3], la, lb);
  hipLaunchKernelGGL(ssim_map_kernel, dim3((unsigned)n_blocks, (unsigned)n_views), dim3(256), 0, s, la, lb, W, H, partial);
  hipLaunchKernelGGL(ssim_finalize_kernel, dim3((unsigned)((n_views + 63) / 64)), dim3(64), 0, s, partial, n_views,
                     n_blocks, (double)(W - 4) * (double)(H - 4), out);
  return hipGetLastError();
}

hipError_t launch_score_finalize(const double* partial, int n_views, int n_blocks, int method,
                                 size_t pixels_per_view, double coverage_weight, prv_score_record* rec, hipStream_t s) {
  hipLaunchKernelGGL(score_finalize_kernel, dim3((unsigned)((n_views + 63) / 64)), dim3(64), 0, s, partial,
                     n_views, n_blocks, method, pixels_per_view, coverage_weight, rec);
  return hipGetLastError();
}

hipError_t launch_synth_table(uint16_t* table, size_t n, uint64_t seed, float amp, hipStream_t s) {
  hipLaunchKernelGGL(synth_table_kernel, dim3(2048), dim3(256), 0, s, table, n, (unsigned long long)seed, amp);
  return hipGetLastError();
}

hipError_t launch_repack_level(const uint16_t* canon, uint16_t* phys, const RepackLevel& L, int F, hipStream_t s) {
  unsigned blocks = ((L.hashed ? L.n : L.res * L.res * L.res) + 255) / 256;
  if (blocks > 8192) blocks = 8192;
  if (blocks == 0) return hipSuccess;
  if (F == 4)
    hipLaunchKernelGGL(repack_level_kernel<4>, dim3(blocks), dim3(256), 0, s, canon, phys, L);
  else
    hipLaunchKernelGGL(repack_level_kernel<2>, dim3(blocks), dim3(256), 0, s, canon, phys, L);
  return hipGetLastError();
}

hipError_t launch_debug_raygen(const CamDev& cam, int W, int H, int spp_k, float* o, float* d, float* t,
                               hipStream_t s) {
  hipLaunchKernelGGL(debug_raygen_kernel, dim3((unsigned)((W * H + 255) / 256)), dim3(256), 0, s, cam, W, H,
                     spp_k, o, d, t);
  return hipGetLastError();
}

hipError_t launch_debug_field(const FieldDev& fd, const float* pos, const float* dir, int n, uint16_t* feat,
                              float* out36, int32_t* occ, hipStream_t s) {
  const unsigned blocks64 = (unsigned)((n + 255) / 256);
  with_field_instance(fd, [&](auto f, auto nd) {
    hipLaunchKernelGGL((debug_field64_kernel<decltype(f)::value, decltype(nd)::value>), dim3(blocks64), dim3(256), 0, s, fd, pos, dir, n, feat, out36, occ);
  });
  return hipGetLastError();
}

}
```

### nerf_prv_amd/csrc/prv_kernels.hpp

```cpp
#pragma once
#include "../../include/prv.h"
#include "prv_device.hpp"
#include <type_traits>

namespace prv {

constexpr size_t kRecordBytes = 96;
constexpr int kRecordWords = 6;
constexpr uint32_t kClaim = 64;
constexpr int kMaxSamples = 128;
constexpr int kNgpMaxSteps = PRV_NGP_MAX_STEPS;
constexpr int kExtChunks = kNgpMaxSteps / 128 - 1;
constexpr size_t kExtBytes = (size_t)kExtChunks * 16;

struct MarchParams {
  FieldDev field;
  const CamDev* cams;
  const int* view_ids;
  int W, H, S;
  uint32_t tiles_x, tiles_y;
  int tile_w_log2, tile_h_log2;
  int spp_inner_log2;
  int live_grid;
  uint32_t live_tiles_max;
// ... 47 lines not shown
bool march_multi_supported(int n_members);
hipError_t launch_march_multi(const MarchMultiParams& P, int n_views, int n_spp, hipStream_t s);
hipError_t launch_occ_interleave(const OccInterleaveParams& P, hipStream_t s);

struct RenderParams {
  FieldDev field;
  const void* queue;
  const uint4* queue_ext;
  int step_mode;
  const uint32_t* queue_count;
  uint32_t* queue_head;
  int n_segments;
  int n_sub;
  uint32_t seg_cap;
  unsigned long long* stat_evaluated;
  float* out_f32;
  uint32_t* out_u8;
  float min_T;
  int last_pass;
  int merge_max;
  int pool_on;
  int cell_cache;
  float bg[4];
};

enum : int { kRenderColour = 0, kRenderDepth = 1, kRenderEntropy = 2, kRenderFootprint = 3, kRenderSurface = 4, kRenderTermination = 5 };

template <int MODE>
struct RenderMode {
  static constexpr bool FOOT = MODE == kRenderFootprint, SURF = MODE == kRenderSurface, TERM = MODE == kRenderTermination;
  static constexpr bool DEPTH = MODE == kRenderDepth || FOOT;
  static constexpr bool ENTROPY = MODE == kRenderEntropy || FOOT || SURF || TERM;
  static constexpr bool DSTATE = DEPTH || SURF;
  static constexpr int kDWord = ENTROPY ? 4 : 6;
  static constexpr int kMoveWords = kDWord + (DSTATE || TERM ? 1 : 0);
  static constexpr int kFrags = ENTROPY ? 8 : kNumFrags;
};
static_assert(RenderMode<kRenderColour>::kMoveWords == 6 && RenderMode<kRenderDepth>::kMoveWords == 7 && RenderMode<kRenderEntropy>::kMoveWords == 4, "moved words");
static_assert(RenderMode<kRenderFootprint>::kMoveWords == 5 && RenderMode<kRenderSurface>::kMoveWords == 5 && RenderMode<kRenderTermination>::kMoveWords == 5, "moved words");

struct RenderPlanesParams {
  RenderParams r;
  float* out_depth;
  const CamDev* cams;
  const int* view_ids;
  uint32_t npix;
  uint32_t nb;
  float* out_entropy;
  float* out_alpha;
  float T_cross;
  float* out_hit;
  float* out_bins;
  size_t plane_stride;
  uint32_t bin_mul;
  uint32_t n_bins;
};

struct EnsembleParams {
  const uint32_t* imgs[PRV_MAX_MODELS];
  int E;
  int view0;
  size_t pixels_per_view;
  double* partial;
};

struct PsnrParams {
  const float* rgba;
  const float* gt;
  const CamDev* cams;
  int W;
  size_t pixels_per_view;
  float bg[4];
  double* partial;
};

struct RepackLevel {
  uint32_t canon_off, phys_off, n, res, sx, hashed;
};
hipError_t launch_repack_level(const uint16_t* canon, uint16_t* phys, const RepackLevel& L, int F, hipStream_t s);

hipError_t launch_march(const MarchParams& P, int n_views, int n_spp, hipStream_t s);
hipError_t launch_spp_reduce(const float* stage, size_t n_pixels, int spp, const float bg[4], float* out, uint32_t* out_u8,
                             hipStream_t s);
hipError_t launch_render(const RenderParams& P, int n_blocks, hipStream_t s);
hipError_t launch_render_planes(const RenderPlanesParams& P, int mode, int n_blocks, hipStream_t s);
hipError_t launch_spp_reduce_depth(const float* stage, size_t n_pixels, int spp, float* out, hipStream_t s);
hipError_t launch_score_entropy(const float* entropy, const float* alpha, size_t npix, int n_views, int n_blocks, double* partial,
                                hipStream_t s);
struct TerminationJsdParams {
  const float* bins[PRV_MAX_MODELS];
  const float* alpha[PRV_MAX_MODELS];
  int E, n_bins;
  size_t npix, plane_stride;
  float* out_jsd;
  double* partial;
};
hipError_t launch_score_termination_jsd(const TerminationJsdParams& P, int n_views, int n_blocks, hipStream_t s);
inline int render_instance_dense_levels(const FieldDev& fd) {
  const int n = fd.n_dense_levels;
  if (!fd.hash_shared) return 0;
  if (fd.n_features == 4) return n == 5 ? 5 : n == 3 ? 3 : 0;
  return n == 10 ? 10 : n == 6 ? 6 : 0;
}
template <class Fn>
void with_field_instance(const FieldDev& fd, Fn&& fn) {
  using std::integral_constant;
  const int nd = render_instance_dense_levels(fd);
  if (fd.n_features == 4) {
    if (nd == 5) fn(integral_constant<int, 4>{}, integral_constant<int, 5>{});
    else if (nd == 3) fn(integral_constant<int, 4>{}, integral_constant<int, 3>{});
    else fn(integral_constant<int, 4>{}, integral_constant<int, 0>{});
  } else {
    if (nd == 10) fn(integral_constant<int, 2>{}, integral_constant<int, 10>{});
    else if (nd == 6) fn(integral_constant<int, 2>{}, integral_constant<int, 6>{});
    else fn(integral_constant<int, 2>{}, integral_constant<int, 0>{});
  }
}
struct PreceptPose {
  double w2c[16], c2w[16];
};
hipError_t launch_precept(const FieldDev& fd, const float* voxels, int n, const PreceptPose& pose, const Rs2Intr& in,
                          float max_range, int32_t* out, hipStream_t s);
hipError_t launch_first_hit(const FieldDev& fd, const CamDev* cams, int n_views, int W, int H, float max_range,
                            int32_t* out, hipStream_t s);
hipError_t launch_splat_points(const float* xyz, const uint8_t* rgb, size_t n, float scale, const float off[3],
                               const CamDev* cams, int n_views, int W, int H, int point_size, int flip180,
                               unsigned long long* zbuf, uint32_t* out, hipStream_t s);
hipError_t launch_quantize(const float* in, size_t n, const float bg[4], uint8_t* out, hipStream_t s);
hipError_t launch_score_ensemble(const EnsembleParams& P, int method, int n_views, int n_blocks, prv_score_record* rec,
                                 hipStream_t s);
hipError_t launch_score_psnr(const PsnrParams& P, int n_views, int n_blocks, hipStream_t s);
hipError_t launch_ssim(const float* img, const float* gt, int n_views, int W, int H, const float bg[4], float* la,
                       float* lb, double* partial, int n_blocks, double* out, hipStream_t s);
hipError_t launch_score_finalize(const double* partial, int n_views, int n_blocks, int method,
                                 size_t pixels_per_view, double coverage_weight, prv_score_record* rec, hipStream_t s);
hipError_t launch_synth_table(uint16_t* table, size_t n, uint64_t seed, float amp, hipStream_t s);
hipError_t launch_debug_raygen(const CamDev& cam, int W, int H, int spp_k, float* o, float* d, float* t,
                               hipStream_t s);
hipError_t launch_debug_field(const FieldDev& fd, const float* pos, const float* dir, int n, uint16_t* feat,
                              float* out36, int32_t* occ, hipStream_t s);

}
```

Before: 24.47 billion.

## Add dense replicas of first hashed grid levels for direct-indexed lookup

At model install, the first few hashed levels after the dense levels are expanded into dense, row-padded 3D grid replicas within a memory budget. The render kernel then indexes these replicas linearly instead of computing XOR hashes, so the eight corner fetches fall in contiguous rows and cache locality improves. The cost is extra device memory (up to 256 MB by default), a fill pass whenever a model is loaded, and additional kernel instantiations.

After: 25.96 billion, median of 6. 1.06x the previous value.

```diff
diff --git a/include/prv.h b/include/prv.h
--- a/include/prv.h
+++ b/include/prv.h
@@ -347,6 +347,8 @@
   int32_t n_dense_levels;
 } prv_model_layout;
 int prv_debug_model_layout(prv_ctx* ctx, int model_slot, prv_model_layout* out);
+int prv_debug_replica_layout(prv_ctx* ctx, int model_slot, int32_t* n_levels, uint64_t* bytes);
+int prv_debug_replica_level(uint32_t res, uint32_t n_features, uint32_t* row_entries, uint64_t* z_stride_bytes, uint64_t* bytes);
 int prv_debug_render_clock(prv_ctx* ctx, uint64_t* shader_cycles, uint64_t* ref_ticks, double* ref_hz);
 int prv_debug_raygen(prv_ctx* ctx, const prv_camset* cs, int view, int width, int height,
                      int spp_index, float* o, float* d, float* t);
diff --git a/nerf_prv_amd/_lib.py b/nerf_prv_amd/_lib.py
--- a/nerf_prv_amd/_lib.py
+++ b/nerf_prv_amd/_lib.py
@@ -245,6 +245,8 @@
     "prv_model_exchange": (_i, [_vp, _vp, _i, C.POINTER(FieldDesc)]),
     "prv_model_exchange_slots": (_i, [_vp, _vp, _i, _P(_i), _P(_i), C.POINTER(FieldDesc)]),
     "prv_debug_model_layout": (_i, [_vp, _i, C.POINTER(ModelLayout)]),
+    "prv_debug_replica_layout": (_i, [_vp, _i, C.POINTER(C.c_int32), C.POINTER(C.c_uint64)]),
+    "prv_debug_replica_level": (_i, [C.c_uint32, C.c_uint32, C.POINTER(C.c_uint32), C.POINTER(C.c_uint64), C.POINTER(C.c_uint64)]),
     "prv_debug_render_clock": (_i, [_vp, C.POINTER(C.c_uint64), C.POINTER(C.c_uint64), C.POINTER(C.c_double)]),
     "prv_debug_raygen": (_i, [_vp, _vp, _i, _i, _i, _i, _vp, _vp, _vp]),
     "prv_debug_mesh_stages": (_i, [_vp, _P(C.c_float)]),
diff --git a/nerf_prv_amd/api.py b/nerf_prv_amd/api.py
--- a/nerf_prv_amd/api.py
+++ b/nerf_prv_amd/api.py
@@ -15,6 +15,19 @@
                  density_bias=3.0, table_amp=4.0)
 FIELD_HBM = dict(n_levels=16, n_features=2, log2_hashmap=24, base_res=16, finest_res=2048, occ_res=128,
                  density_bias=3.0, table_amp=4.0)
+
+
+def replica_level(res, n_features=4):
+    row, mz, b = C.c_uint32(), C.c_uint64(), C.c_uint64()
+    if L.load().prv_debug_replica_level(int(res), int(n_features), C.byref(row), C.byref(mz), C.byref(b)) != 0:
+        raise PrvError(L.PRV_E_INVALID, "prv_debug_replica_level failed")
+    return row.value, mz.value, b.value
+
+
+def replica_layout(ctx, model_slot):
+    n, b = C.c_int32(), C.c_uint64()
+    ctx._chk(ctx.lib.prv_debug_replica_layout(ctx.handle, int(model_slot), C.byref(n), C.byref(b)))
+    return n.value, b.value
 
 
 class RenderMode(enum.IntEnum):
diff --git a/nerf_prv_amd/csrc/prv_api.cpp b/nerf_prv_amd/csrc/prv_api.cpp
--- a/nerf_prv_amd/csrc/prv_api.cpp
+++ b/nerf_prv_amd/csrc/prv_api.cpp
@@ -47,6 +47,9 @@
   uint64_t phys_bytes = 0;
   float occ_lo[3] = {0, 0, 0}, occ_hi[3] = {1, 1, 1};
   Buffer table, phys, occ, occ_coarse, frags, frags64, mlp;
+  Buffer repl;
+  ReplicaDev rdev{};
+  uint64_t repl_bytes = 0;
 };
 
 }
@@ -212,6 +215,43 @@
 }
 const float kSynthSpheres[4][4] = {
     {0.50f, 0.50f, 0.50f, 0.35f}, {0.80f, 0.50f, 0.62f, 0.13f}, {0.36f, 0.80f, 0.45f, 0.11f}, {0.40f, 0.24f, 0.78f, 0.10f}};
+
+constexpr uint64_t kReplicaBudgetDefault = (uint64_t)256 << 20;
+
+int build_replicas(prv_ctx* c, Model& m) {
+  const FieldDev& f = m.dev;
+  m.rdev = ReplicaDev{};
+  m.repl_bytes = 0;
+  int cap = kMaxReplicas;
+  uint64_t budget = kReplicaBudgetDefault;
+  if (const char* e = getenv("PRV_REPLICA_LEVELS")) cap = std::max(0, std::min(kMaxReplicas, atoi(e)));
+  if (const char* e = getenv("PRV_REPLICA_MB")) budget = (uint64_t)std::max(0ll, std::min(strtoll(e, nullptr, 10), 1ll << 20)) << 20;
+  int n = 0;
+  uint64_t total = 0;
+  uint32_t pack[kMaxReplicas] = {0, 0, 0};
+  if (f.n_features == 4 && render_instance_dense_levels(f) == 5) {
+    for (int l = f.n_dense_levels; l < f.n_levels && n < cap; l++, n++) {
+      const uint32_t res = f.levels[l].res_m1 + 1u;
+      const ReplicaLevelLayout lay = replica_level_layout(res, 8u);
+      if (res > 1024u || lay.bytes == 0 || total + lay.bytes > budget || total + lay.bytes >= (1ull << 32)) break;
+      pack[n] = (uint32_t)total | (lay.row / 8u);
+      total += lay.bytes;
+    }
+  }
+  if (n == 0) {
+    m.repl.reset();
+    return PRV_OK;
+  }
+  int rc;
+  if ((rc = ensure(c, m.repl, total)) != PRV_OK) return rc;
+  m.rdev.table = (const uint16_t*)m.repl.p;
+  m.rdev.n_levels = n;
+  memcpy(m.rdev.pack, pack, sizeof(pack));
+  m.repl_bytes = total;
+  for (int k = 0; k < n; k++) HIPCHK(c, launch_fill_replica(f, m.rdev, k, c->stream));
+  HIPCHK(c, hipStreamSynchronize(c->stream));
+  return PRV_OK;
+}
 
 int install_model(prv_ctx* c, int slot, const prv_field_desc& d, const uint16_t* mlp, const uint32_t* occ_host,
                   const uint16_t* table_host ) {
@@ -400,6 +440,7 @@
       L.pack = (L.off_b & ~31u) | (sx[l] & 31u);
     }
   }
+  if ((rc = build_replicas(c, m)) != PRV_OK) return rc;
   m.loaded = true;
   m.dirty = false;
   return PRV_OK;
@@ -830,7 +871,7 @@
       pp.bin_mul = (uint32_t)(n_bins * 65536u / (size_t)(ngp ? kNgpMaxSteps : o->samples_per_ray));
     }
     if ((rc = timed(c, c->ev_render, [&] {
-           HIPCHK(c, n_planes ? launch_render_planes(pp, t.mode, n_blocks, c->stream) : launch_render(pp.r, n_blocks, c->stream));
+           HIPCHK(c, n_planes ? launch_render_planes(pp, t.mode, n_blocks, c->stream) : launch_render(pp.r, m.rdev, n_blocks, c->stream));
            return PRV_OK;
          })) != PRV_OK)
       return rc;
@@ -931,7 +972,7 @@
     const int n_blocks = render_blocks(c, m, npix);
     uint32_t* q_head = (uint32_t*)((char*)c->counters_multi.p + (size_t)e * kStatOffset);
     const RenderParams rp = render_params(c, m, o, L, mp.seg_cap, mp.mem[e], q_head, stat, kRenderColour);
-    if ((rc = timed(c, c->ev_render, [&] { HIPCHK(c, launch_render(rp, n_blocks, c->stream)); return PRV_OK; })) != PRV_OK) return rc;
+    if ((rc = timed(c, c->ev_render, [&] { HIPCHK(c, launch_render(rp, m.rdev, n_blocks, c->stream)); return PRV_OK; })) != PRV_OK) return rc;
     if (spp > 1)
       HIPCHK(c, launch_spp_reduce((const float*)mp.mem[e].out_f32, (size_t)n_views * npix, spp, o->background, scratch_f32, (uint32_t*)out_u8[e], c->stream));
   }
@@ -2025,6 +2066,26 @@
   return PRV_OK;
 } catch (...) { return caught(c); }
 
+int prv_debug_replica_layout(prv_ctx* c, int slot, int32_t* n_levels, uint64_t* bytes) try {
+  if (!c) return PRV_E_INVALID;
+  int rc = check_model(c, slot);
+  if (rc != PRV_OK) return rc;
+  if (!n_levels || !bytes) return fail(c, PRV_E_INVALID, "out is NULL");
+  const Model& m = c->models[slot];
+  *n_levels = replica_instance_levels(m.dev, m.rdev);
+  *bytes = m.repl_bytes;
+  return PRV_OK;
+} catch (...) { return caught(c); }
+
+int prv_debug_replica_level(uint32_t res, uint32_t n_features, uint32_t* row_entries, uint64_t* z_stride_bytes, uint64_t* bytes) {
+  if (!row_entries || !z_stride_bytes || !bytes || res < 1 || res > 4096 || (n_features != 2 && n_features != 4)) return PRV_E_INVALID;
+  const ReplicaLevelLayout lay = replica_level_layout(res, n_features * 2u);
+  *row_entries = lay.row;
+  *z_stride_bytes = (uint64_t)lay.row * lay.row * n_features * 2u;
+  *bytes = lay.bytes;
+  return PRV_OK;
+}
+
 int prv_debug_raygen(prv_ctx* c, const prv_camset* cs, int view, int W, int H, int spp_k, float* o, float* d, float* t) try {
   if (!c) return PRV_E_INVALID;
   if (!cs || view < 0 || view >= (int)cs->cams.size() || W < 1 || H < 1 || !o || !d || !t)
@@ -2058,7 +2119,7 @@
     return rc;
   HIPCHK(c, hipMemcpyAsync(c->dbg[0].p, pos, N * 12, hipMemcpyHostToDevice, c->stream));
   if (dir) HIPCHK(c, hipMemcpyAsync(c->dbg[1].p, dir, N * 12, hipMemcpyHostToDevice, c->stream));
-  HIPCHK(c, launch_debug_field(c->models[slot].dev, (const float*)c->dbg[0].p, dir ? (const float*)c->dbg[1].p : nullptr,
+  HIPCHK(c, launch_debug_field(c->models[slot].dev, c->models[slot].rdev, (const float*)c->dbg[0].p, dir ? (const float*)c->dbg[1].p : nullptr,
                                n, (uint16_t*)c->dbg[3].p, (float*)c->dbg[4].p, (int32_t*)c->dbg[5].p, c->stream));
   if (feat) HIPCHK(c, hipMemcpyAsync(feat, c->dbg[3].p, N * 64, hipMemcpyDeviceToHost, c->stream));
   if (out36) HIPCHK(c, hipMemcpyAsync(out36, c->dbg[4].p, N * 144, hipMemcpyDeviceToHost, c->stream));
diff --git a/nerf_prv_amd/csrc/prv_device.hpp b/nerf_prv_amd/csrc/prv_device.hpp
--- a/nerf_prv_amd/csrc/prv_device.hpp
+++ b/nerf_prv_amd/csrc/prv_device.hpp
@@ -41,6 +41,13 @@
   int wide_offsets;
   float density_bias;
   float occ_lo[3], occ_hi[3];
+};
+
+constexpr int kMaxReplicas = 3;
+struct ReplicaDev {
+  const uint16_t* table;
+  uint32_t pack[kMaxReplicas];
+  int n_levels;
 };
 
 struct CamDev {
@@ -291,7 +298,7 @@
   uint32_t my_b, mz_b, m_b;
   uint32_t wide;
 };
-enum { kLevelDense = 0, kLevelHashedShared = 1, kLevelGeneric = 2 };
+enum { kLevelDense = 0, kLevelHashedShared = 1, kLevelGeneric = 2, kLevelReplica = 3 };
 
 template <int F>
 struct CornerCache {
@@ -316,9 +323,10 @@
   uint32_t vw[8][F / 2];
   uint32_t pk = L.pack;
   if (KIND != kLevelGeneric) asm volatile("" : "+s"(pk));
-  if (DENSE) {
-    const uint32_t sxl = pk & 31u, off = pk & ~31u;
-    const uint32_t my = (uint32_t)(F * 2) << sxl, mz = (uint32_t)(F * 2) << (2u * sxl);
+  if (DENSE || KIND == kLevelReplica) {
+    const uint32_t sxl = pk & 31u, row8 = pk & 4095u, off = pk & (DENSE ? ~31u : ~4095u);
+    const uint32_t my = DENSE ? (uint32_t)(F * 2) << sxl : row8 * (uint32_t)(F * 16);
+    const uint32_t mz = DENSE ? (uint32_t)(F * 2) << (2u * sxl) : my * (row8 << 3);
     const char* base0 = reinterpret_cast<const char*>(table) + off;
     const char* base1 = base0 + my;
     const uint32_t b = (c0[0] << ESH) + __umul24(c0[1], my) + __umul24(c0[2], mz);
@@ -486,21 +494,36 @@
                : blend_level<F>(cc[J >= NDENSE ? J - NDENSE : 0].v, hwa[J >= NDENSE ? J - NDENSE : 0], out + J * (F / 2))), ...);
 }
 
-template <int F, int NDENSE, int... J>
+template <int F, int NDENSE, int NREPL, int J>
+__device__ __forceinline__ void encode_level_at(const uint16_t* __restrict__ table, const LevelDev* __restrict__ lv, const HashConsts& H,
+                                                const ReplicaDev* __restrict__ R, float px, float py, float pz, half2v* out) {
+  if constexpr (J >= NDENSE && J < NDENSE + NREPL) {
+    LevelDev L = {};
+    L.scale = lv[J].scale;
+    L.pack = R->pack[J - NDENSE];
+    encode_level2<F, kLevelReplica>(R->table, L, H, px, py, pz, out + J * (F / 2));
+  } else {
+    encode_level2<F, (J < NDENSE ? kLevelDense : NDENSE > 0 ? kLevelHashedShared : kLevelGeneric)>(table, lv[J], H, px, py, pz, out + J * (F / 2));
+  }
+}
+template <int F, int NDENSE, int NREPL, int... J>
 __device__ __forceinline__ void encode_all_levels(const uint16_t* __restrict__ table, const LevelDev* __restrict__ lv, const HashConsts& H,
-                                                  float px, float py, float pz, half2v* out, std::integer_sequence<int, J...>) {
-  (encode_level2<F, (J < NDENSE ? kLevelDense : NDENSE > 0 ? kLevelHashedShared : kLevelGeneric)>(table, lv[J], H, px, py, pz, out + J * (F / 2)), ...);
-}
-
-template <int F, int NDENSE, bool CACHE = false>
+                                                  const ReplicaDev* __restrict__ R, float px, float py, float pz, half2v* out,
+                                                  std::integer_sequence<int, J...>) {
+  (encode_level_at<F, NDENSE, NREPL, J>(table, lv, H, R, px, py, pz, out), ...);
+}
+
+template <int F, int NDENSE, bool CACHE = false, int NREPL = 0>
 __device__ __forceinline__ void encode_sample(const uint16_t* __restrict__ table, const LevelDev* __restrict__ lv, const HashConsts& H,
-                                              float px, float py, float pz, half8 f[4], CornerCache<F>* cc = nullptr) {
+                                              float px, float py, float pz, half8 f[4], CornerCache<F>* cc = nullptr,
+                                              const ReplicaDev* __restrict__ R = nullptr) {
+  static_assert(NREPL == 0 || (!CACHE && NDENSE > 0 && NDENSE + NREPL <= 32 / F && NREPL <= kMaxReplicas), "replicas: plain instances with dense levels only");
   px = clamp01(px);
   py = clamp01(py);
   pz = clamp01(pz);
   half2v out[16];
   if constexpr (CACHE && NDENSE > 0) encode_all_levels_cached<F, NDENSE>(table, lv, H, px, py, pz, out, cc, std::make_integer_sequence<int, 32 / F>{});
-  else encode_all_levels<F, NDENSE>(table, lv, H, px, py, pz, out, std::make_integer_sequence<int, 32 / F>{});
+  else encode_all_levels<F, NDENSE, NREPL>(table, lv, H, R, px, py, pz, out, std::make_integer_sequence<int, 32 / F>{});
 #pragma unroll
   for (int s = 0; s < 4; s++)
 #pragma unroll
diff --git a/nerf_prv_amd/csrc/prv_kernels.hip b/nerf_prv_amd/csrc/prv_kernels.hip
--- a/nerf_prv_amd/csrc/prv_kernels.hip
+++ b/nerf_prv_amd/csrc/prv_kernels.hip
@@ -586,8 +586,8 @@
 
 __device__ __forceinline__ float entropy_add(float p, float H) { return p >= 1.17549435e-38f ? fmaf(p, -__builtin_amdgcn_logf(p), H) : H; }
 
-template <int F, int NDENSE, bool NGP, bool CACHE, int MODE>
-__device__ __forceinline__ void render_queue64_body(RenderParams P, const RenderPlanesParams* X) {
+template <int F, int NDENSE, bool NGP, bool CACHE, int MODE, int NREPL = 0>
+__device__ __forceinline__ void render_queue64_body(RenderParams P, const RenderPlanesParams* X, const ReplicaDev* R = nullptr) {
   using M = RenderMode<MODE>;
   constexpr int kDWord = M::kDWord, kMoveWords = M::kMoveWords, kFrags = M::kFrags;
   __shared__ half8 wl[kFrags * 64];
@@ -884,7 +884,7 @@
       const float t = fmaf((float)i + 0.5f, dt, t0);
       if constexpr (M::DSTATE) ts = t;
       if constexpr (M::TERM) sbin = min((i * X->bin_mul) >> 16, X->n_bins - 1u);
-      encode_sample<F, NDENSE, CACHE>(P.field.table, lvl, hc, fmaf(t, d[0], o[0]), fmaf(t, d[1], o[1]), fmaf(t, d[2], o[2]), f, cc);
+      encode_sample<F, NDENSE, CACHE, NREPL>(P.field.table, lvl, hc, fmaf(t, d[0], o[0]), fmaf(t, d[1], o[1]), fmaf(t, d[2], o[2]), f, cc, R);
     }
     swap_halves(f[0], f[1]);
     swap_halves(f[2], f[3]);
@@ -961,6 +961,13 @@
 __attribute__((amdgpu_waves_per_eu(CACHE ? 2 : NDENSE == 0 ? 1 : 3)))
 void render_queue64_kernel(RenderParams P) {
   render_queue64_body<F, NDENSE, NGP, CACHE, kRenderColour>(P, nullptr);
+}
+
+template <bool NGP, int NREPL>
+__global__ __launch_bounds__(256)
+__attribute__((amdgpu_waves_per_eu(3)))
+void render_queue64_replica_kernel(RenderParams P, ReplicaDev R) {
+  render_queue64_body<4, 5, NGP, false, kRenderColour, NREPL>(P, nullptr, &R);
 }
 
 template <int F, int NDENSE, bool NGP, int MODE>
@@ -1457,6 +1464,27 @@
   }
 }
 
+template <int F>
+__global__ __launch_bounds__(256) void fill_replica_kernel(const uint16_t* __restrict__ phys, uint16_t* __restrict__ repl, uint32_t level_pack,
+                                                           HashConsts H, uint32_t replica_pack, uint32_t res) {
+  typedef typename EntryWord<F>::type word_t;
+  constexpr int ESH = F == 4 ? 3 : 2;
+  const uint32_t res_m1 = level_pack & 4095u, n1 = res + 1u;
+  const char* src = reinterpret_cast<const char*>(phys) + (level_pack & ~4095u);
+  const uint32_t row8 = replica_pack & 4095u;
+  const uint32_t my = row8 * (uint32_t)(F * 16), mz = my * (row8 << 3);
+  char* dst = reinterpret_cast<char*>(repl) + (replica_pack & ~4095u);
+  const uint32_t nv = n1 * n1 * n1;
+  for (uint32_t i = blockIdx.x * 256 + threadIdx.x; i < nv; i += gridDim.x * 256) {
+    const uint32_t x = i % n1, y = (i / n1) % n1, z = i / (n1 * n1);
+    const uint32_t tx = min(x, res_m1) << ESH;
+    const uint32_t ty = __umul24(min(y, res_m1), H.my_b) & H.m_b;
+    const uint32_t tz = __umul24(min(z, res_m1), H.mz_b) & H.m_b;
+    const word_t v = *reinterpret_cast<const word_t*>(src + (tx ^ ty ^ tz));
+    *reinterpret_cast<word_t*>(dst + ((x << ESH) + __umul24(y, my) + __umul24(z, mz))) = v;
+  }
+}
+
 
 __global__ __launch_bounds__(256) void debug_raygen_kernel(CamDev cam, int W, int H, int spp_k,
                                                            float* __restrict__ o_out,
@@ -1477,10 +1505,10 @@
   t_out[i * 2 + 1] = t1;
 }
 
-template <int F, int NDENSE>
+template <int F, int NDENSE, int NREPL = 0>
 __global__ __launch_bounds__(256) void debug_field64_kernel(FieldDev fd, const float* __restrict__ pos, const float* __restrict__ dir,
                                                             int n, uint16_t* __restrict__ feat, float* __restrict__ out36,
-                                                            int32_t* __restrict__ occ_out) {
+                                                            int32_t* __restrict__ occ_out, ReplicaDev R) {
   __shared__ half8 wl[kNumFrags * 64];
   const LevelDev* __restrict__ lvl = fd.levels;
   for (int i = threadIdx.x; i < kNumFrags * 64; i += 256) wl[i] = fd.frags64[i];
@@ -1502,7 +1530,7 @@
   dir_of(idxB, dB);
   half8 f[4];
   const HashConsts hc = {fd.hash_my_b, fd.hash_mz_b, fd.hash_m_b, (uint32_t)fd.wide_offsets};
-  encode_sample<F, NDENSE>(fd.table, lvl, hc, p[0], p[1], p[2], f);
+  encode_sample<F, NDENSE, false, NREPL>(fd.table, lvl, hc, p[0], p[1], p[2], f, nullptr, NREPL > 0 ? &R : nullptr);
   if (ok && feat) {
     typedef uint16_t ushort8 __attribute__((ext_vector_type(8)));
     uint16_t* dst = feat + (size_t)idx * 32;
@@ -1642,19 +1670,30 @@
 }
 
 template <bool NGP>
-static void launch_render_mode(const RenderParams& P, int n_blocks, hipStream_t s) {
+static void launch_render_mode(const RenderParams& P, const ReplicaDev& R, int n_blocks, hipStream_t s) {
   if (P.cell_cache && P.field.n_features == 4 && render_instance_dense_levels(P.field) == 5) {
     hipLaunchKernelGGL((render_queue64_kernel<4, 5, NGP, true>), dim3(n_blocks), dim3(256), 0, s, P);
     return;
   }
+  if (const int nr = NGP ? std::min(replica_instance_levels(P.field, R), kReplicaLevelsNgp) : replica_instance_levels(P.field, R)) {
+    if constexpr (!NGP) {
+      if (nr == 3) {
+        hipLaunchKernelGGL((render_queue64_replica_kernel<false, 3>), dim3(n_blocks), dim3(256), 0, s, P, R);
+        return;
+      }
+    }
+    if (nr >= 2) hipLaunchKernelGGL((render_queue64_replica_kernel<NGP, 2>), dim3(n_blocks), dim3(256), 0, s, P, R);
+    else hipLaunchKernelGGL((render_queue64_replica_kernel<NGP, 1>), dim3(n_blocks), dim3(256), 0, s, P, R);
+    return;
+  }
   with_field_instance(P.field, [&](auto f, auto nd) {
     hipLaunchKernelGGL((render_queue64_kernel<decltype(f)::value, decltype(nd)::value, NGP>), dim3(n_blocks), dim3(256), 0, s, P);
   });
 }
 
-hipError_t launch_render(const RenderParams& P, int n_blocks, hipStream_t s) {
-  if (P.step_mode == PRV_STEP_NGP) launch_render_mode<true>(P, n_blocks, s);
-  else launch_render_mode<false>(P, n_blocks, s);
+hipError_t launch_render(const RenderParams& P, const ReplicaDev& R, int n_blocks, hipStream_t s) {
+  if (P.step_mode == PRV_STEP_NGP) launch_render_mode<true>(P, R, n_blocks, s);
+  else launch_render_mode<false>(P, R, n_blocks, s);
   return hipGetLastError();
 }
 
@@ -1753,6 +1792,16 @@
   return hipGetLastError();
 }
 
+hipError_t launch_fill_replica(const FieldDev& fd, const ReplicaDev& R, int k, hipStream_t s) {
+  const LevelDev& L = fd.levels[fd.n_dense_levels + k];
+  const uint32_t res = L.res_m1 + 1u, nv = (res + 1u) * (res + 1u) * (res + 1u);
+  if (fd.n_features != 4 || k < 0 || k >= R.n_levels || res > 1024u) return hipErrorInvalidValue;
+  const HashConsts hc = {fd.hash_my_b, fd.hash_mz_b, fd.hash_m_b, 0u};
+  hipLaunchKernelGGL(fill_replica_kernel<4>, dim3(std::min(8192u, (nv + 255u) / 256u)), dim3(256), 0, s, fd.table,
+                     const_cast<uint16_t*>(R.table), L.pack, hc, R.pack[k], res);
+  return hipGetLastError();
+}
+
 hipError_t launch_repack_level(const uint16_t* canon, uint16_t* phys, const RepackLevel& L, int F, hipStream_t s) {
   unsigned blocks = ((L.hashed ? L.n : L.res * L.res * L.res) + 255) / 256;
   if (blocks > 8192) blocks = 8192;
@@ -1771,11 +1820,17 @@
   return hipGetLastError();
 }
 
-hipError_t launch_debug_field(const FieldDev& fd, const float* pos, const float* dir, int n, uint16_t* feat,
+hipError_t launch_debug_field(const FieldDev& fd, const ReplicaDev& R, const float* pos, const float* dir, int n, uint16_t* feat,
                               float* out36, int32_t* occ, hipStream_t s) {
   const unsigned blocks64 = (unsigned)((n + 255) / 256);
+  if (const int nr = replica_instance_levels(fd, R)) {
+    if (nr == 3) hipLaunchKernelGGL((debug_field64_kernel<4, 5, 3>), dim3(blocks64), dim3(256), 0, s, fd, pos, dir, n, feat, out36, occ, R);
+    else if (nr == 2) hipLaunchKernelGGL((debug_field64_kernel<4, 5, 2>), dim3(blocks64), dim3(256), 0, s, fd, pos, dir, n, feat, out36, occ, R);
+    else hipLaunchKernelGGL((debug_field64_kernel<4, 5, 1>), dim3(blocks64), dim3(256), 0, s, fd, pos, dir, n, feat, out36, occ, R);
+    return hipGetLastError();
+  }
   with_field_instance(fd, [&](auto f, auto nd) {
-    hipLaunchKernelGGL((debug_field64_kernel<decltype(f)::value, decltype(nd)::value>), dim3(blocks64), dim3(256), 0, s, fd, pos, dir, n, feat, out36, occ);
+    hipLaunchKernelGGL((debug_field64_kernel<decltype(f)::value, decltype(nd)::value>), dim3(blocks64), dim3(256), 0, s, fd, pos, dir, n, feat, out36, occ, R);
   });
   return hipGetLastError();
 }
diff --git a/nerf_prv_amd/csrc/prv_kernels.hpp b/nerf_prv_amd/csrc/prv_kernels.hpp
--- a/nerf_prv_amd/csrc/prv_kernels.hpp
+++ b/nerf_prv_amd/csrc/prv_kernels.hpp
@@ -153,7 +153,7 @@
 hipError_t launch_march(const MarchParams& P, int n_views, int n_spp, hipStream_t s);
 hipError_t launch_spp_reduce(const float* stage, size_t n_pixels, int spp, const float bg[4], float* out, uint32_t* out_u8,
                              hipStream_t s);
-hipError_t launch_render(const RenderParams& P, int n_blocks, hipStream_t s);
+hipError_t launch_render(const RenderParams& P, const ReplicaDev& R, int n_blocks, hipStream_t s);
 hipError_t launch_render_planes(const RenderPlanesParams& P, int mode, int n_blocks, hipStream_t s);
 hipError_t launch_spp_reduce_depth(const float* stage, size_t n_pixels, int spp, float* out, hipStream_t s);
 hipError_t launch_score_entropy(const float* entropy, const float* alpha, size_t npix, int n_views, int n_blocks, double* partial,
@@ -187,6 +187,21 @@
     else fn(integral_constant<int, 2>{}, integral_constant<int, 0>{});
   }
 }
+constexpr int kReplicaLevelsNgp = 2;
+inline int replica_instance_levels(const FieldDev& fd, const ReplicaDev& R) {
+  return R.table && fd.n_features == 4 && render_instance_dense_levels(fd) == 5 ? R.n_levels : 0;
+}
+struct ReplicaLevelLayout {
+  uint32_t row;
+  uint64_t bytes;
+};
+inline ReplicaLevelLayout replica_level_layout(uint32_t res, uint32_t ebytes) {
+  const uint32_t row = (res + 1u + 7u) & ~7u;
+  const uint64_t mz = (uint64_t)row * row * ebytes;
+  if (mz >= (1ull << 24) || row / 8u > 4095u) return {row, 0};
+  return {row, (mz * (res + 1u) + 4095ull) & ~4095ull};
+}
+hipError_t launch_fill_replica(const FieldDev& fd, const ReplicaDev& R, int k, hipStream_t s);
 struct PreceptPose {
   double w2c[16], c2w[16];
 };
@@ -208,7 +223,7 @@
 hipError_t launch_synth_table(uint16_t* table, size_t n, uint64_t seed, float amp, hipStream_t s);
 hipError_t launch_debug_raygen(const CamDev& cam, int W, int H, int spp_k, float* o, float* d, float* t,
                                hipStream_t s);
-hipError_t launch_debug_field(const FieldDev& fd, const float* pos, const float* dir, int n, uint16_t* feat,
+hipError_t launch_debug_field(const FieldDev& fd, const ReplicaDev& R, const float* pos, const float* dir, int n, uint16_t* feat,
                               float* out36, int32_t* occ, hipStream_t s);
 
 }
```
